# JosephCatrambone/aruco3

Measured on AMD Instinct MI355X. Metric: frames/sec at 1920x1080 ARUCO dict, higher is better.
Workload: dtype u8

## Files before the change

aruco3_amd/csrc/a3_api.hip:

```cpp
#include <algorithm>
#include <atomic>
#include <cmath>
#include <chrono>
#include <cstddef>
#include <cstdio>
#include <cstring>
#include <mutex>
#include <string>
#include <vector>

#include "a3_common.h"
#include "a3_internal.h"

namespace a3 {
hipError_t launch_grey_threshold(hipStream_t, const uint8_t*, int, size_t, size_t, int, int, uint32_t, uint32_t, uint8_t*, uint64_t*, uint16_t*);
bool threshold_writes_grey_plane(uint32_t radius, const uint8_t* pixels, size_t row_stride, size_t frame_stride, int W);
hipError_t launch_dart_count(hipStream_t, const uint64_t*, int, int, uint32_t, uint32_t, unsigned long long*, uint32_t*, uint64_t, uint32_t*, uint32_t*, void*, size_t);
size_t tile_darts_bytes(uint32_t W, uint32_t H, uint32_t n_frames);
size_t tile_off_offset(uint32_t W, uint32_t H, uint32_t n_frames);
size_t tile_mask_offset_bytes(uint32_t W, uint32_t H, uint32_t n_frames);
hipError_t launch_dart_build(hipStream_t, const uint64_t*, int, int, uint32_t, uint32_t, const uint32_t*, const uint32_t*, uint32_t*, const uint32_t*,
                             uint64_t*, uint32_t*, uint32_t, const uint32_t*, int, const unsigned long long*);
hipError_t launch_zero(hipStream_t, void*, size_t);
size_t entry_state_bytes();
bool finalize_inline(bool frame_entries, bool trust_natural);
size_t fin_state_bytes();
size_t entry_slots(uint32_t);
size_t leader_list_bytes(uint32_t);
hipError_t launch_rank_cycles(hipStream_t, uint32_t, int, const uint64_t*, const uint32_t*,
                              uint32_t*, unsigned int*, void*, void*, void*, uint32_t*, unsigned int*, int, DeviceCounters*, const uint32_t*, int,
                              const uint32_t*, uint32_t*, uint32_t, int, uint32_t, unsigned int*, int);
hipError_t launch_resolve(hipStream_t, const void*, uint32_t, int, const uint64_t*, const uint32_t*, const unsigned int*, uint64_t*, uint64_t*,
                          DeviceCounters*, int, const uint32_t*);
hipError_t launch_select_scatter(hipStream_t, const void*, uint32_t, const uint32_t*, const unsigned int*, const uint32_t*, const uint64_t*,
                                 const uint32_t*, uint32_t, uint32_t,
                                 uint32_t, double, double, ContourRec*, uint32_t*, uint32_t, uint64_t, DeviceCounters*,
                                 const uint64_t*, uint32_t*, const uint32_t*, int, uint32_t*, int, const void*);
hipError_t launch_debug_clockwise(hipStream_t, const int32_t*, uint32_t, int32_t*);
hipError_t launch_unpack_bits(hipStream_t, const uint64_t*, int, int, uint8_t*);
hipError_t launch_contour_quads(hipStream_t, const ContourRec*, const DeviceCounters*, uint32_t, const uint32_t*, double, uint32_t, uint32_t,
                                uint32_t, CandRec*, uint32_t*, unsigned int*, int, uint32_t);
size_t decode_out_bytes();
hipError_t launch_frame_candidates(hipStream_t, const CandRec*, const uint32_t*, uint32_t, uint32_t, float, uint16_t*, uint16_t*, uint32_t*,
                                   uint32_t*, unsigned int*, uint32_t, void*, float*);
uint32_t frame_cand_lds_slots();
size_t proj_rec_bytes();
size_t weight_table_bytes();
hipError_t launch_weight_table(hipStream_t, uint32_t, uint32_t, uint32_t, float*);
hipError_t launch_decode(hipStream_t, PixelSrc, int, int, uint32_t, const uint16_t*, const uint32_t*, const unsigned int*, uint32_t,
                         uint32_t, uint32_t, uint32_t, const uint64_t*, uint32_t, uint32_t, int, void*, const float*, void*, uint8_t*, uint32_t, uint32_t*, int, int, int);
hipError_t launch_compact_markers(hipStream_t, const void*, const uint16_t*, const uint32_t*, uint32_t, uint32_t, uint32_t, a3_marker*,
                                  uint32_t, uint32_t*, unsigned int*, unsigned int*, const uint32_t*, unsigned int*);
hipError_t launch_pack_detections(hipStream_t, const a3_marker*, const a3_pose*, const uint32_t*, uint32_t, uint32_t, uint32_t, void*, unsigned int*);
hipError_t launch_debug_rotate_bits(hipStream_t, const uint8_t*, uint32_t, uint32_t, uint8_t*);
hipError_t launch_gather_patches(hipStream_t, const void*, uint32_t, const uint8_t*, uint32_t, uint32_t, uint8_t*, unsigned int*);
hipError_t launch_pose(hipStream_t, const uint32_t*, uint32_t, const float*, uint32_t, const unsigned int*, int, float, float, float, float,
                       float, float, float, a3_pose*);
hipError_t launch_find_nearest(hipStream_t, const uint64_t*, uint32_t, const uint64_t*, uint32_t, uint32_t*, uint8_t*);
size_t refine_params_bytes();
void refine_params(void*, const a3_refine_config&, uint32_t);
hipError_t launch_refine_corners(hipStream_t, PixelSrc, uint32_t, uint32_t, const a3_marker*, const unsigned int*, const float*, const float*, uint32_t,
                                 const void*, float*);
size_t board_slot_bytes();
void board_slot_from(const float*, void*);
hipError_t launch_board_pose(hipStream_t, const a3_marker*, const uint32_t*, const float*, const float*, const unsigned int*, const uint32_t*,
                             uint32_t, uint32_t, const uint16_t*, uint32_t, const void*, const a3_intrinsics*, uint32_t, uint32_t, a3_board_pose*);
hipError_t launch_undistort_corners(hipStream_t, const a3_marker*, const float*, const unsigned int*, uint32_t, const a3_intrinsics&,
                                    const a3_distortion&, float*, float*);
hipError_t launch_charuco_corners(hipStream_t, PixelSrc, uint32_t, uint32_t, const a3_marker*, const uint32_t*, const float*, const float*,
                                  const unsigned int*, const uint32_t*, uint32_t, uint32_t, const uint16_t*, uint32_t, const void*, const float*,
                                  const uint32_t*, uint32_t, uint32_t, uint32_t, const void*, const a3_intrinsics*, const a3_distortion*,
                                  a3_charuco_corner*, uint32_t*, a3_charuco_corner*, float*);
hipError_t launch_charuco_pose(hipStream_t, const a3_marker*, const float*, const unsigned int*, const uint32_t*, uint32_t, uint32_t, const uint16_t*,
                               uint32_t, const void*, const float*, uint32_t, const uint32_t*, const a3_charuco_corner*, const float*,
                               const a3_intrinsics*, uint32_t, uint32_t, a3_charuco_pose*);
hipError_t launch_calc_tau(hipStream_t, const uint64_t*, uint32_t, unsigned int*);
size_t rig_obs_bytes();
size_t rig_frame_bytes();
size_t rig_table_bytes();
hipError_t launch_rig(hipStream_t, const a3_rig*, uint32_t, const a3_rig_camera*, const a3_rig_observation*, const float*, const float*, uint32_t*,
                      double*, double*, a3_rig_result*, a3_rig_camera_result*, a3_rig_frame*, a3_rig_observation_result*);
size_t calib_view_bytes();
hipError_t launch_calibrate(hipStream_t, const a3_calib_camera*, uint32_t, const uint32_t*, const float*, const float*, double*, a3_calib_result*,
                            a3_calib_view*);
hipError_t launch_synth_render(hipStream_t, const a3_synth_frame*, uint32_t, const a3_synth_marker*, uint32_t, uint32_t, int, float, float, int,
                               uint8_t*, size_t, size_t);
hipError_t launch_spin(hipStream_t, int, int, int, uint32_t*);
hipError_t launch_selftest(hipStream_t, const double*, const double*, uint32_t, double*, double*, float*, float*);
}

using namespace a3;

namespace {

thread_local std::string g_create_error;

constexpr uint32_t kMaxCandDefault = 1024, kMaxCandLimit = A3_MAX_CANDIDATES_PER_FRAME;
static_assert(kMaxCandLimit == 65536, "a3_marker.candidate_index is a uint16_t");
constexpr uint32_t kMaxContoursDefault = 1u << 20;
constexpr uint64_t kMaxDartsDefault = 48ull << 20;
constexpr uint64_t kMaxPointsDefault = 64ull << 20;
constexpr uint64_t kHardMaxDarts = (1ull << 30) - (1ull << 16);
constexpr uint64_t kHardMaxPoints = 3ull << 30;
constexpr int kResolveItersMax = 16;
constexpr uint32_t kPatchCapMin = 32768, kPatchCapMax = 1u << 20;

struct DevBuf {
    void* p = nullptr;
    size_t cap = 0;
    hipError_t ensure(size_t bytes) {
        if (bytes <= cap) return hipSuccess;
        if (p) { hipError_t e = hipFree(p); p = nullptr; cap = 0; if (e != hipSuccess) return e; }
        hipError_t e = hipMalloc(&p, bytes);
        if (e == hipSuccess) cap = bytes;
        return e;
    }
    void release() { if (p) (void)hipFree(p); p = nullptr; cap = 0; }
    template <typename T> T* as() const { return reinterpret_cast<T*>(p); }
};

struct Chunk { uint32_t first, count; uint64_t darts; uint32_t max_frame_darts; };
struct Batch {
    const uint8_t* pixels = nullptr; int fmt = 0;
    uint32_t W = 0, H = 0, n = 0;
    size_t row_stride = 0, frame_stride = 0, out_cap = 0;
    bool want_pose = false, pose_has_intr = false;
    float pose_size_mm = 0.0f;
    a3_intrinsics pose_intr{};
    size_t pose_bytes = 0;
    a3_refine_config refine{};
    size_t refine_bytes = 0;
    bool board = false;
// ... 202 lines not shown
bool g_hold_rests = true;
std::atomic<int> g_jump_rounds_cap{0};
enum { kStreamCopy = 0, kStreamDecode = 1 };

hipError_t create_stream(hipStream_t* st) { return hipStreamCreateWithPriority(st, hipStreamNonBlocking, 0); }

hipError_t device_stream(int device, int kind, hipStream_t* out) {
    std::lock_guard<std::mutex> lk(g_streams_mu);
    DeviceStreams& ds = g_dev_streams[device & 63];
    hipStream_t& st = kind == kStreamDecode ? ds.decode : ds.copy;
    if (!st) {
        const hipError_t e = create_stream(&st);
        if (e != hipSuccess) { st = nullptr; return e; }
    }
    *out = st;
    return hipSuccess;
}

int need_stream(a3_ctx* ctx);

std::mutex g_defer_mu;
std::vector<a3_ctx*> g_deferred;
std::atomic<int> g_overlap_force{-1};
std::vector<a3_ctx*> g_contexts;
int batch_mode_of(const a3_ctx* ctx) {
    const int f = g_overlap_force.load(std::memory_order_relaxed);
    if (f >= 0) return f;
    if (!ctx->stream || ctx->stream == ctx->own_stream) return 0;
    std::lock_guard<std::mutex> lk(g_streams_mu);
    for (const a3_ctx* o : g_contexts)
        if (o != ctx && o->device == ctx->device && o->stream == ctx->stream) return 2;
    return 0;
}
int release_mode() {
    const int f = g_overlap_force.load(std::memory_order_relaxed);
    return f >= 0 ? f : 2;
}

const void* refine_params_for(a3_ctx* ctx, const a3_refine_config& cfg) {
    if (ctx->refine_prm.empty() || memcmp(&ctx->refine_prm_cfg, &cfg, sizeof cfg) != 0) {
        ctx->refine_prm.assign((refine_params_bytes() + 3) / 4, 0.0f);
        refine_params(ctx->refine_prm.data(), cfg, ctx->mark_size);
        ctx->refine_prm_cfg = cfg;
    }
    return ctx->refine_prm.data();
}

size_t charuco_slot_bytes(const Batch& b) { return ((size_t)b.n * b.charuco_nc * sizeof(a3_charuco_corner) + 255) & ~(size_t)255; }
size_t charuco_stage_off(const Batch& b) {
    return b.head_bytes + (size_t)b.guess * (sizeof(a3_marker) + b.pose_bytes + b.refine_bytes + b.undist_bytes) +
           (b.board ? (size_t)b.n * sizeof(a3_board_pose) : 0);
}
size_t charuco_stage_bytes(const Batch& b) {
    return b.charuco ? 16 + (size_t)b.charuco_guess * sizeof(a3_charuco_corner) + (b.want_pose ? (size_t)b.n * sizeof(a3_charuco_pose) : 0) : 0;
}
const void* charuco_params_for(a3_ctx* ctx, const a3_charuco_config& cfg) {
    if (ctx->charuco_prm.empty() || memcmp(&ctx->charuco_prm_cfg, &cfg, sizeof cfg) != 0) {
        ctx->charuco_prm.assign((refine_params_bytes() + 3) / 4, 0.0f);
        const a3_refine_config rc{A3_REFINE_SUBPIX, cfg.win_half, cfg.relative_win, cfg.max_iterations, cfg.min_shift};
        refine_params(ctx->charuco_prm.data(), rc, 0);
        ctx->charuco_prm_cfg = cfg;
    }
    return ctx->charuco_prm.data();
}

int enqueue_back(a3_ctx* ctx, hipStream_t st, const Batch& b) {
    const uint32_t S = ctx->cfg.homography_sample_size;
    const float min_corner_separation = (float)std::min(b.W, b.H) * ctx->cfg.min_corner_separation_factor;
    unsigned int* d_work_count = ctx->scratch_u32 + 0;
    unsigned int* d_marker_total = ctx->scratch_u32 + 1;
    unsigned int* d_err = ctx->scratch_u32 + 4;
    if (ctx->inject_armed) {
        ctx->inject_armed = false;
        const uint32_t cnt = (uint32_t)ctx->inject.size();
        if (cnt) A3_HIP(hipMemcpyAsync(ctx->cands.p, ctx->inject.data(), cnt * sizeof(CandRec), hipMemcpyHostToDevice, st));
        ctx->inject_count = cnt;
        A3_HIP(hipMemcpyAsync(ctx->cand_count, &ctx->inject_count, 4, hipMemcpyHostToDevice, st));
    }
    A3_HIP(launch_frame_candidates(st, ctx->cands.as<CandRec>(), ctx->cand_count, b.n, b.max_cand, min_corner_separation,
                                   ctx->pre_xy.as<uint16_t>(), ctx->fin_xy.as<uint16_t>(), ctx->fin_count.as<uint32_t>(),
                                   ctx->work.as<uint32_t>(), d_work_count, S, ctx->proj.p, ctx->cand_big.as<float>()));
    const int few = b.n <= 64u ? 1 : 0;
    A3_HIP(launch_decode(st, b.src, (int)b.W, (int)b.H, 0, ctx->fin_xy.as<uint16_t>(), ctx->work.as<uint32_t>(), d_work_count,
                         b.max_cand, S, ctx->mark_size, S, ctx->dict.as<uint64_t>(), ctx->n_codes, ctx->tau, ctx->cfg.filter_high_bit_errors,
                         ctx->proj.p, ctx->wtab.as<float>(), ctx->outs.p, b.taps ? ctx->patches.as<uint8_t>() : nullptr, b.patch_cap, ctx->per_frame,
                         (int)std::min<uint32_t>(4096u, b.n * 128u) , 0,
                         few));
    A3_HIP(launch_compact_markers(st, ctx->outs.p, ctx->fin_xy.as<uint16_t>(), ctx->fin_count.as<uint32_t>(), b.n, 0, b.max_cand,
                                  ctx->markers_ptr, b.marker_cap, ctx->per_frame, d_marker_total, d_err, ctx->cand_count, ctx->scratch_u32 + 2));
    if (b.refine_bytes)
        A3_HIP(launch_refine_corners(st, b.src, b.W, b.H, ctx->markers_ptr, d_marker_total, nullptr, nullptr, b.marker_cap,
                                     refine_params_for(ctx, b.refine), ctx->refined_buf.as<float>()));
    if (b.undist_bytes)
        A3_HIP(launch_undistort_corners(st, ctx->markers_ptr, b.refine_bytes ? ctx->refined_buf.as<float>() : nullptr, d_marker_total, b.marker_cap,
                                        b.pose_intr, b.dist, ctx->undist_buf.as<float>(), ctx->undist_buf.as<float>() + (size_t)b.marker_cap * 8));
    const float* fcorners = b.undist_bytes ? ctx->undist_buf.as<float>() : b.refine_bytes ? ctx->refined_buf.as<float>() : nullptr;
    const uint32_t* charuco_counts = b.charuco ? reinterpret_cast<const uint32_t*>(ctx->charuco_tmp.as<uint8_t>() + charuco_slot_bytes(b)) : nullptr;
    float* charuco_und = b.charuco && b.want_pose && b.undist_bytes ? ctx->charuco_und.as<float>() : nullptr;
    if (b.charuco)
        A3_HIP(launch_charuco_corners(st, b.src, b.W, b.H, ctx->markers_ptr, nullptr, nullptr, b.refine_bytes ? ctx->refined_buf.as<float>() : nullptr,
                                      d_marker_total, ctx->per_frame, b.marker_cap, b.n, ctx->board_slot_of.as<uint16_t>(), ctx->n_codes,
                                      ctx->board_slot_rec.p, ctx->charuco_tab.as<float>(), ctx->charuco_tab.as<uint32_t>() + 2 * (size_t)b.charuco_nc,
                                      b.charuco_nc, b.charuco_cfg.min_markers, b.charuco_cfg.refine, charuco_params_for(ctx, b.charuco_cfg),
                                      &b.pose_intr, &b.dist, ctx->charuco_tmp.as<a3_charuco_corner>(), const_cast<uint32_t*>(charuco_counts),
                                      ctx->charuco_buf.as<a3_charuco_corner>(), charuco_und));
    if (b.want_pose) {
        const a3_intrinsics& in = b.pose_intr;
        if (fcorners)
            A3_HIP(launch_pose(st, nullptr, 8u, fcorners, b.marker_cap, d_marker_total, b.pose_has_intr ? 4 : 3, b.pose_size_mm,
                               (float)b.W, (float)b.H, in.focal_x, in.focal_y, in.principal_x, in.principal_y, ctx->pose_buf.as<a3_pose>()));
        else
            A3_HIP(launch_pose(st, reinterpret_cast<const uint32_t*>(reinterpret_cast<const uint8_t*>(ctx->markers_ptr) + offsetof(a3_marker, corners)),
                               (uint32_t)(sizeof(a3_marker) / 4), nullptr, b.marker_cap, d_marker_total, b.pose_has_intr ? 1 : 0, b.pose_size_mm,
                               (float)b.W, (float)b.H, in.focal_x, in.focal_y, in.principal_x, in.principal_y, ctx->pose_buf.as<a3_pose>()));
        if (b.board)
            A3_HIP(launch_board_pose(st, ctx->markers_ptr, nullptr, nullptr, fcorners, d_marker_total,
                                     ctx->per_frame, b.marker_cap, b.n, ctx->board_slot_of.as<uint16_t>(), ctx->n_codes, ctx->board_slot_rec.p,
                                     b.pose_has_intr ? &in : nullptr, b.W, b.H, ctx->board_buf.as<a3_board_pose>()));
        if (b.charuco)
            A3_HIP(launch_charuco_pose(st, ctx->markers_ptr, fcorners, d_marker_total, ctx->per_frame, b.marker_cap, b.n,
                                       ctx->board_slot_of.as<uint16_t>(), ctx->n_codes, ctx->board_slot_rec.p, ctx->charuco_tab.as<float>(),
                                       b.charuco_nc, charuco_counts, ctx->charuco_buf.as<a3_charuco_corner>(), charuco_und,
                                       b.pose_has_intr ? &in : nullptr, b.W, b.H, ctx->charuco_pose_buf.as<a3_charuco_pose>()));
    }
    if (b.prof >= 2) A3_HIP(hipEventRecord(ctx->ev[3], st));
    uint8_t* hp = (uint8_t*)ctx->pinned;
    a3_pose* h_poses = reinterpret_cast<a3_pose*>(hp + b.head_bytes + (size_t)b.guess * sizeof(a3_marker));
    A3_HIP(hipMemcpyAsync(hp, ctx->scratch_u32, b.head_bytes + (size_t)b.guess * sizeof(a3_marker), hipMemcpyDeviceToHost, st));
    if (b.pose_bytes) A3_HIP(hipMemcpyAsync(h_poses, ctx->pose_buf.p, (size_t)b.guess * b.pose_bytes, hipMemcpyDeviceToHost, st));
    if (b.refine_bytes)
        A3_HIP(hipMemcpyAsync(reinterpret_cast<uint8_t*>(h_poses) + (size_t)b.guess * b.pose_bytes, ctx->refined_buf.p, (size_t)b.guess * b.refine_bytes,
                              hipMemcpyDeviceToHost, st));
    if (b.board)
        A3_HIP(hipMemcpyAsync(reinterpret_cast<uint8_t*>(h_poses) + (size_t)b.guess * (b.pose_bytes + b.refine_bytes), ctx->board_buf.p,
                              (size_t)b.n * sizeof(a3_board_pose), hipMemcpyDeviceToHost, st));
    if (b.undist_bytes) {
        uint8_t* hu = reinterpret_cast<uint8_t*>(h_poses) + (size_t)b.guess * (b.pose_bytes + b.refine_bytes) + (b.board ? (size_t)b.n * sizeof(a3_board_pose) : 0);
        A3_HIP(hipMemcpyAsync(hu, ctx->undist_buf.p, (size_t)b.guess * 32, hipMemcpyDeviceToHost, st));
        A3_HIP(hipMemcpyAsync(hu + (size_t)b.guess * 32, ctx->undist_buf.as<float>() + (size_t)b.marker_cap * 8, (size_t)b.guess * 16,
                              hipMemcpyDeviceToHost, st));
    }
    if (b.charuco) {
        uint8_t* hc = hp + charuco_stage_off(b);
        A3_HIP(hipMemcpyAsync(hc, charuco_counts + b.n, 4, hipMemcpyDeviceToHost, st));
        A3_HIP(hipMemcpyAsync(hc + 16, ctx->charuco_buf.p, (size_t)b.charuco_guess * sizeof(a3_charuco_corner), hipMemcpyDeviceToHost, st));
        if (b.want_pose)
            A3_HIP(hipMemcpyAsync(hc + 16 + (size_t)b.charuco_guess * sizeof(a3_charuco_corner), ctx->charuco_pose_buf.p,
                                  (size_t)b.n * sizeof(a3_charuco_pose), hipMemcpyDeviceToHost, st));
    }
    if (b.taps) {
        A3_HIP(hipMemcpyAsync(ctx->pinned_counts, ctx->cand_count, (size_t)b.n * 4, hipMemcpyDeviceToHost, st));
        A3_HIP(hipMemcpyAsync((uint8_t*)ctx->pinned_counts + (size_t)b.n * 4, ctx->fin_count.p, (size_t)b.n * 4, hipMemcpyDeviceToHost, st));
    }
    A3_HIP(hipEventRecord(ctx->ev[4], st));
    return A3_OK;
}

int flush_deferred_impl(a3_ctx* ctx, hipEvent_t after);
int flush_deferred_locked(a3_ctx* ctx, hipEvent_t after) {
    const int rc = flush_deferred_impl(ctx, after);
    if (rc) ctx->back_rc = rc;
    return rc;
}
int flush_deferred_impl(a3_ctx* ctx, hipEvent_t after) {
    if (!ctx->back_deferred) return A3_OK;
    ctx->back_deferred = false;
    for (size_t i = 0; i < g_deferred.size(); i++)
// ... 193 lines not shown
        ctx->per_frame = reinterpret_cast<uint32_t*>(z + head_off + 256 + ctr_bytes);
        ctx->markers_ptr = reinterpret_cast<a3_marker*>(z + head_off + head_bytes);
        zero_p = z; zero_bytes = (head_off + head_bytes + 15) & ~(size_t)15;
        return launch ? launch_zero(st, zero_p, zero_bytes) : hipSuccess;
    };
    std::vector<Chunk> chunks;
    std::vector<uint64_t> fd;
    if (device_plan) {
        if (int rc = ensure_chain_buffers(ctx, st, b, cap_d)) return rc;
        chunks.push_back(Chunk{0, n, cap_d, (uint32_t)std::min<uint64_t>(cap_d, 0xFFFFFFFFu)});
        A3_HIP(layout_zero_block(1, n, false));
        ctx->frame_darts_ptr = ctx->frame_darts_dev.as<unsigned long long>();
    } else {
        A3_HIP(ctx->tile_darts.ensure(tile_darts_bytes(W, H, n)));
        ctx->frame_darts_ptr = ctx->frame_darts.as<unsigned long long>();
        A3_HIP(hipMemsetAsync(ctx->frame_darts.p, 0, (size_t)n * 8, st));
    }
    A3_HIP(launch_dart_count(st, ctx->bin.as<uint64_t>(), (int)W, (int)H, 0, n, ctx->frame_darts_ptr, ctx->tile_darts.as<uint32_t>(), cap_d,
                             device_plan ? ctx->frame_base.as<uint32_t>() : nullptr, device_plan ? ctx->scratch_u32 + 8 : nullptr,
                             device_plan ? zero_p : nullptr, device_plan ? zero_bytes : 0));
    const uint32_t* n_live = device_plan ? ctx->scratch_u32 + 8 : nullptr;
    uint32_t max_chunk_frames = n;
    if (!device_plan) {
        if (int rc = ensure_pinned(ctx, std::max<size_t>((size_t)n * 8, 1 << 16))) return rc;
        A3_HIP(hipMemcpyAsync(ctx->pinned, ctx->frame_darts.p, (size_t)n * 8, hipMemcpyDeviceToHost, st));
        A3_HIP(wait_stream(st));
        fd.assign((uint64_t*)ctx->pinned, (uint64_t*)ctx->pinned + n);
        uint64_t biggest = 0;
        for (uint64_t v : fd) { biggest = std::max(biggest, v); ctx->stats.darts += v; }
        if (biggest > kHardMaxDarts) return fail(ctx, A3_ERR_LIMIT, "a frame needs more contour-graph nodes than 32-bit indices allow");
        if (biggest > ctx->max_darts) ctx->max_darts = biggest;
        Chunk c{0, 0, 0, 0};
        for (uint32_t f = 0; f < n; f++) {
            if (c.count && (c.darts + fd[f] > ctx->max_darts || c.count >= kMaxChunkFrames)) { chunks.push_back(c); c = Chunk{f, 0, 0, 0}; }
            c.count++; c.darts += fd[f]; c.max_frame_darts = (uint32_t)std::max<uint64_t>(c.max_frame_darts, fd[f]);
        }
        if (c.count) chunks.push_back(c);
        max_chunk_frames = 0; uint64_t max_chunk_darts = 0;
        for (auto& c : chunks) { max_chunk_frames = std::max(max_chunk_frames, c.count); max_chunk_darts = std::max(max_chunk_darts, c.darts); }
        if (int rc = ensure_dart_pool(ctx, pool_darts_of(ctx, max_chunk_darts, chunks.size()))) return rc;
        A3_HIP(ctx->pix_base.ensure((size_t)max_chunk_frames * npx * 4));
        A3_HIP(ctx->frame_base.ensure((size_t)(max_chunk_frames + 1) * 4 * chunks.size()));
        A3_HIP(layout_zero_block(chunks.size(), max_chunk_frames, true));
        A3_HIP(ctx->contours.ensure((size_t)ctx->max_contours * sizeof(ContourRec)));
        A3_HIP(ctx->cyc_start_off.ensure((size_t)ctx->max_contours * 4));
        A3_HIP(ctx->points.ensure(ctx->max_points * 4));
        std::vector<uint32_t> bases;
        for (auto& c : chunks) {
            uint32_t acc = 0;
            for (uint32_t i = 0; i < max_chunk_frames + 1; i++) {
                bases.push_back(acc);
                if (i < c.count) acc += (uint32_t)fd[c.first + i];
            }
        }
        if (int rc = ensure_pinned(ctx, (size_t)n * 8 + bases.size() * 4 + (1 << 16))) return rc;
        uint32_t* h_bases = reinterpret_cast<uint32_t*>((uint8_t*)ctx->pinned + (size_t)n * 8);
        memcpy(h_bases, bases.data(), bases.size() * 4);
        A3_HIP(hipMemcpyAsync(ctx->frame_base.p, h_bases, bases.size() * 4, hipMemcpyHostToDevice, st));
    }
    ctx->stats.chunks = (uint32_t)chunks.size();

    unsigned int* d_err = ctx->scratch_u32 + 4;
    unsigned int* d_entry_count = ctx->scratch_u32 + 32;
    unsigned int* d_leader_count = ctx->scratch_u32 + 16;
    unsigned int* d_dead_count = ctx->scratch_u32 + 48;

    const uint64_t* d_bin = ctx->bin.as<uint64_t>();
    const double image_diag = std::sqrt((double)W * W + (double)H * H);
    const double eps_factor = ctx->cfg.contour_simplification_epsilon;
    const int resolve_iters = ctx->resolve_full_ttl > 0 ? ctx->resolve_iters_hint : 0;
    const int inline_resolve_W = ctx->resolve_full_ttl > 0 ? 0 : (int)W;
    const int keep_all = b.taps ? 1 : 0;
    int rounds_max = 0;
    for (size_t ci = 0; ci < chunks.size(); ci++) {
        const Chunk& c = chunks[ci];
        DeviceCounters* ctr = ctx->counters + ci;
        const uint32_t* fb = ctx->frame_base.as<uint32_t>() + ci * (max_chunk_frames + 1);
        const uint32_t nd = (uint32_t)c.darts;
        if (nd == 0) continue;
        if (ci > 0) {
            A3_HIP(hipMemsetAsync(d_leader_count, 0, 4 * 32, st));
            A3_HIP(hipMemsetAsync(ctx->frame_cursor, 0, (size_t)c.count * 4, st));
        }
        const uint32_t* tile_off = ctx->tile_darts.as<uint32_t>() + tile_off_offset(W, H, n);
        A3_HIP(launch_dart_build(st, d_bin, (int)W, (int)H, c.first, c.count, fb, tile_off, ctx->pix_base.as<uint32_t>(),
                                 ctx->tile_darts.as<uint32_t>(), ctx->d_xy.as<uint64_t>(), ctx->d_succ.as<uint32_t>(), nd, n_live, 0,
                                 reinterpret_cast<const unsigned long long*>(ctx->tile_darts.as<uint8_t>() + tile_mask_offset_bytes(W, H, n))));
        int rounds = 1;
        while ((1ull << rounds) < (uint64_t)c.max_frame_darts && rounds < 31) rounds++;
        rounds += 1;
        rounds = std::min(rounds, ctx->jump_rounds_hint);
        if (const int cap = g_jump_rounds_cap.load(std::memory_order_relaxed); cap > 0 && ctx->jump_rounds_hint < 32) rounds = std::min(rounds, cap);
        rounds_max = std::max(rounds_max, rounds);
        uint32_t* const frame_entries = ctx->entry_global_ttl > 0 ? nullptr : ctx->frame_cursor;
        const bool dense_graph = (uint64_t)nd * 10u >= (uint64_t)c.count * npx;
        unsigned int* const dead_ctr = (keep_all || !dense_graph) ? nullptr : d_dead_count;
        A3_HIP(launch_rank_cycles(st, nd, (int)W, ctx->d_xy.as<uint64_t>(), ctx->d_succ.as<uint32_t>(),
                                  ctx->entry_list.as<uint32_t>(), d_entry_count, ctx->es_a.p, ctx->es_b.p,
                                  ctx->fin.p, ctx->leader_list.as<uint32_t>(), d_leader_count, rounds, ctr, n_live, 0, fb,
                                  frame_entries, c.count, 1, min_edge_length, dead_ctr, inline_resolve_W > 0 ? 1 : 0));
        if (rel_mode == 2) { if (int rc = release_waiting()) return rc; }
        ctx->dbg_nd = nd; ctx->dbg_frames = c.count; ctx->dbg_chunks = (uint32_t)chunks.size();
        A3_HIP(launch_rank_cycles(st, nd, (int)W, ctx->d_xy.as<uint64_t>(), ctx->d_succ.as<uint32_t>(),
                                  ctx->entry_list.as<uint32_t>(), d_entry_count, ctx->es_a.p, ctx->es_b.p,
                                  ctx->fin.p , ctx->leader_list.as<uint32_t>(), d_leader_count, rounds, ctr,
                                  n_live, 0, fb, frame_entries, c.count, 2, min_edge_length, dead_ctr, inline_resolve_W > 0 ? 1 : 0));
        const void* fin = ctx->fin.p;
        A3_HIP(launch_resolve(st, fin, nd, (int)W, ctx->d_xy.as<uint64_t>(), ctx->leader_list.as<uint32_t>(), d_leader_count,
                              ctx->t_cur.as<uint64_t>(), ctx->t_next.as<uint64_t>(), ctr, resolve_iters, n_live));
        A3_HIP(launch_select_scatter(st, fin, nd, ctx->leader_list.as<uint32_t>(), d_leader_count, ctx->d_succ.as<uint32_t>(), ctx->t_cur.as<uint64_t>(), fb,
                                     c.count, c.first, min_edge_length, eps_factor, image_diag,
                                     ctx->contours.as<ContourRec>(), ctx->cyc_start_off.as<uint32_t>(), ctx->max_contours, ctx->max_points, ctr,
                                     ctx->d_xy.as<uint64_t>(), ctx->points.as<uint32_t>(), n_live, inline_resolve_W, ctx->leader_keep.as<uint32_t>(),
                                     keep_all, finalize_inline(frame_entries != nullptr, inline_resolve_W > 0) ? ctx->es_a.p : nullptr));
        A3_HIP(launch_contour_quads(st, ctx->contours.as<ContourRec>(), ctr, ctx->max_contours, ctx->points.as<uint32_t>(),
                                    eps_factor, min_edge_length, c.first, kMaxCand,
                                    ctx->cands.as<CandRec>() + (size_t)c.first * kMaxCand, ctx->cand_count + c.first, d_err,
                                    W <= 16384u && H <= 16384u ? 1 : 0, nd));
    }
    if (rel_mode != 0) { if (int rc = release_waiting()) return rc; }
    if (b.prof >= 2) A3_HIP(hipEventRecord(ctx->ev[2], st));

    b.src = b.need_grey ? PixelSrc{ctx->grey.as<uint8_t>(), W, (unsigned long long)npx, kFmtGreyPlane}
                        : PixelSrc{b.pixels, b.row_stride, b.frame_stride, b.fmt};
    ctx->dbg_src = b.src;
    b.head_bytes = head_bytes;
    if (int rc = ensure_back_buffers(ctx, b, head_bytes)) return rc;
    b.device_plan = device_plan; b.n_chunks = chunks.size(); b.chunk0_darts = chunks.empty() ? 0 : chunks[0].darts;
    b.ctr_bytes = ctr_bytes; b.rounds_max = rounds_max;
    ctx->counts_valid = false;
    if (ctx->allow_defer && !defer_locked && b.profiling < 2 && ctx->batch_mode != 0) {
        A3_HIP(hipEventRecord(ctx->ev_contours, st));
        std::lock_guard<std::mutex> lk(g_defer_mu);
        ctx->back_deferred = true;
        ctx->back_rc = 0;
        ctx->stepping = A3_STEP_DECODE_DEFERRED;
        g_deferred.push_back(ctx);
    } else if (int rc = enqueue_back(ctx, st, b)) return rc;
    b.active = true;
    return A3_OK;
}

int enqueue_batch(a3_ctx* ctx) {
    ctx->stepping = A3_STEP_WHOLE;
    if (int rc = enqueue_front(ctx, ctx->batch, false)) return rc;
    return enqueue_chain(ctx, ctx->batch, false);
}

int finish_batch(a3_ctx* ctx, a3_marker* out, a3_pose* poses, size_t out_cap, uint32_t* per_frame_count, size_t* out_n) {
    Batch& b = ctx->batch;
    if (!b.active) return fail(ctx, A3_ERR_INVALID, "no batch was submitted");
    {
        std::lock_guard<std::mutex> lk(g_defer_mu);
        (void)flush_held_locked(ctx, nullptr);
        if (const int rc = ctx->held_rc) { ctx->held_rc = 0; b.active = false; return rc; }
    }
    b.active = false;
    hipStream_t st = ctx->stream;
    const size_t ctr_bytes = b.ctr_bytes, head_bytes = b.head_bytes, pose_bytes = b.pose_bytes, n_chunks = b.n_chunks, refine_bytes = b.refine_bytes;
    const size_t undist_bytes = b.undist_bytes, board_bytes = b.board ? (size_t)b.n * sizeof(a3_board_pose) : 0;
    const uint32_t guess = b.guess, n = b.n;
    uint8_t* hp = (uint8_t*)ctx->pinned;
    a3_marker* h_markers = reinterpret_cast<a3_marker*>(hp + head_bytes);
    a3_pose* h_poses = reinterpret_cast<a3_pose*>(hp + head_bytes + (size_t)guess * sizeof(a3_marker));
    const float* h_refined = reinterpret_cast<const float*>(hp + head_bytes + (size_t)guess * (sizeof(a3_marker) + pose_bytes));
    const float* h_undist = reinterpret_cast<const float*>(hp + head_bytes + (size_t)guess * (sizeof(a3_marker) + pose_bytes + refine_bytes) + board_bytes);
    const float* h_undist_res = h_undist + (size_t)guess * 8;
    {
        std::lock_guard<std::mutex> lk(g_defer_mu);
        if (int rc = flush_deferred_locked(ctx, nullptr)) return rc;
// ... 543 lines not shown
        ctx->stepping = A3_STEP_BURST_LAST; ctx->released_others = released;
        return erc;
    }
    ctx->allow_defer = true;
    const int erc = enqueue_batch(ctx);
    ctx->allow_defer = false;
    return erc;
}

static int collect_common(a3_ctx* ctx, a3_marker* out, a3_pose* poses, size_t out_cap, uint32_t* per_frame_count, size_t* out_n) {
    *out_n = 0;
    if (ctx->pending_trivial) {
        ctx->pending_trivial = false;
        finish_trivial(ctx, per_frame_count);
        return A3_OK;
    }
    A3_HIP(hipSetDevice(ctx->device));
    if (int rcs_ = need_stream(ctx)) return rcs_;
    int rc = finish_batch(ctx, out, poses, out_cap, per_frame_count, out_n);
    const uint32_t stepping = ctx->stepping;
    if (rc == 1) { ctx->reruns++; ctx->batch.out_cap = out_cap; rc = run_batch_with_retries(ctx, out, poses, out_cap, per_frame_count, out_n); }
    ctx->stepping = stepping;
    return rc;
}

int a3_detect_batch_submit(a3_ctx* ctx, const void* pixels, int memory, int fmt, uint32_t width, uint32_t height, size_t row_stride,
                           size_t frame_stride, uint32_t n_frames, size_t out_cap) {
    if (!ctx) return A3_ERR_INVALID;
    return submit_common(ctx, pixels, memory, fmt, width, height, row_stride, frame_stride, n_frames, out_cap, false, 0.0f, nullptr);
}

int a3_detect_batch_collect(a3_ctx* ctx, a3_marker* out, size_t out_cap, uint32_t* per_frame_count, size_t* out_n) {
    if (!ctx) return A3_ERR_INVALID;
    if (!out_n || (!out && out_cap)) return fail(ctx, A3_ERR_INVALID, "a3_detect_batch_collect: null output");
    return collect_common(ctx, out, nullptr, out_cap, per_frame_count, out_n);
}

int a3_detect_batch_pose_submit(a3_ctx* ctx, const void* pixels, int memory, int fmt, uint32_t width, uint32_t height, size_t row_stride,
                                size_t frame_stride, uint32_t n_frames, float marker_size_mm, const a3_intrinsics* intr, size_t out_cap) {
    if (!ctx) return A3_ERR_INVALID;
    return submit_common(ctx, pixels, memory, fmt, width, height, row_stride, frame_stride, n_frames, out_cap, true, marker_size_mm, intr);
}

int a3_detect_batch_pose_collect(a3_ctx* ctx, a3_marker* out, a3_pose* poses, size_t out_cap, uint32_t* per_frame_count, size_t* out_n) {
    if (!ctx) return A3_ERR_INVALID;
    if (!out_n || (!out && out_cap) || (!poses && out_cap)) return fail(ctx, A3_ERR_INVALID, "a3_detect_batch_pose_collect: null output");
    if (!ctx->pending_trivial && ctx->batch.active && !ctx->batch.want_pose)
        return fail(ctx, A3_ERR_INVALID, "a3_detect_batch_pose_collect: the submitted batch was not an a3_detect_batch_pose_submit call");
    return collect_common(ctx, out, poses, out_cap, per_frame_count, out_n);
}

int a3_detect_batch_pose(a3_ctx* ctx, const void* pixels, int memory, int fmt, uint32_t width, uint32_t height, size_t row_stride,
                         size_t frame_stride, uint32_t n_frames, float marker_size_mm, const a3_intrinsics* intr, a3_marker* out,
                         a3_pose* poses, size_t out_cap, uint32_t* per_frame_count, size_t* out_n) {
    if (!ctx || !poses) return A3_ERR_INVALID;
    return detect_common(ctx, pixels, memory, fmt, width, height, row_stride, frame_stride, n_frames, true, marker_size_mm, intr, out, poses,
                         out_cap, per_frame_count, out_n);
}

int a3_debug_kernel_time(a3_ctx* ctx, int kernel, int dbg, int reps, float* avg_ms) {
    if (!ctx || !avg_ms || reps <= 0) return A3_ERR_INVALID;
    if (ctx->dbg_chunks != 1 || ctx->dbg_nd == 0) return fail(ctx, A3_ERR_INVALID, "needs a preceding single-chunk batch");
    A3_HIP(hipSetDevice(ctx->device));
    if (int rcs_ = need_stream(ctx)) return rcs_;
    hipStream_t st = ctx->stream;
    struct EventPair {
        hipEvent_t e0 = nullptr, e1 = nullptr;
        ~EventPair() { if (e0) (void)hipEventDestroy(e0); if (e1) (void)hipEventDestroy(e1); }
    } evp;
    A3_HIP(hipEventCreate(&evp.e0)); A3_HIP(hipEventCreate(&evp.e1));
    const hipEvent_t e0 = evp.e0, e1 = evp.e1;
    double total = 0.0;
    unsigned int* d_entry_count = ctx->scratch_u32 + 32;
    unsigned int* d_leader_count = ctx->scratch_u32 + 16;
    for (int r = 0; r < reps; r++) {
        A3_HIP(hipMemsetAsync(d_leader_count, 0, 4 * 32, st));
        A3_HIP(hipEventRecord(e0, st));
        if (kernel == 0) {
            A3_HIP(hipMemsetAsync(ctx->frame_darts.p, 0, (size_t)ctx->frames * 8, st));
            A3_HIP(launch_dart_count(st, ctx->bin.as<uint64_t>(), (int)ctx->W, (int)ctx->H, 0, ctx->frames, ctx->frame_darts.as<unsigned long long>(),
                                     ctx->tile_darts.as<uint32_t>(), 0, nullptr, nullptr, nullptr, 0));
        } else if (kernel == 1) {
            A3_HIP(launch_dart_build(st, ctx->bin.as<uint64_t>(), (int)ctx->W, (int)ctx->H, 0, ctx->dbg_frames, ctx->frame_base.as<uint32_t>(),
                                     ctx->tile_darts.as<uint32_t>() + tile_off_offset(ctx->W, ctx->H, ctx->frames), ctx->pix_base.as<uint32_t>(),
                                     ctx->tile_darts.as<uint32_t>(), ctx->d_xy.as<uint64_t>(),
                                     ctx->d_succ.as<uint32_t>(), ctx->dbg_nd, nullptr, dbg ? dbg : 5,
                                     reinterpret_cast<const unsigned long long*>(ctx->tile_darts.as<uint8_t>() + tile_mask_offset_bytes(ctx->W, ctx->H, ctx->frames))));
        } else if (kernel == 2) {
            A3_HIP(launch_rank_cycles(st, ctx->dbg_nd, (int)ctx->W, ctx->d_xy.as<uint64_t>(), ctx->d_succ.as<uint32_t>(),
                                      ctx->entry_list.as<uint32_t>(),
                                      d_entry_count, ctx->es_a.p, ctx->es_b.p, ctx->fin.p,
                                      ctx->leader_list.as<uint32_t>(), d_leader_count, 0, ctx->counters, nullptr, dbg ? dbg : 11, ctx->frame_base.as<uint32_t>(), nullptr, ctx->dbg_frames, 0,
                                      0u, nullptr, 0));
        } else if (kernel == 3 || kernel == 4) {
            if (kernel == 4) {
                const size_t sweep = std::min<size_t>(ctx->pix_base.cap & ~(size_t)15, (size_t)512 << 20);
                if (sweep) A3_HIP(launch_zero(st, ctx->pix_base.p, sweep));
                A3_HIP(hipEventRecord(e0, st));
            }
            A3_HIP(launch_decode(st, ctx->dbg_src, (int)ctx->W, (int)ctx->H, 0, ctx->fin_xy.as<uint16_t>(), ctx->work.as<uint32_t>(), ctx->scratch_u32,
                                 ctx->max_cand, ctx->cfg.homography_sample_size, ctx->mark_size, ctx->cfg.homography_sample_size, ctx->dict.as<uint64_t>(),
                                 ctx->n_codes, ctx->tau, ctx->cfg.filter_high_bit_errors, ctx->proj.p, ctx->wtab.as<float>(), ctx->outs.p, nullptr, 0u, nullptr, 4096,
                                 dbg == 0 ? -1000 : dbg, ctx->frames <= 64u ? 1 : 0));
        } else return fail(ctx, A3_ERR_INVALID, "kernel: 0 dart_count, 1 dart_assign, 2 local_contract, 3 decode, 4 decode on cold frames");
        A3_HIP(hipEventRecord(e1, st));
        A3_HIP(hipStreamSynchronize(st));
        float ms = 0;
        A3_HIP(hipEventElapsedTime(&ms, e0, e1));
        total += ms;
    }
    *avg_ms = (float)(total / reps);
    return A3_OK;
}

int a3_debug_set_overlap(int mode) {
    if (mode < -1 || mode > 2) return A3_ERR_INVALID;
    std::lock_guard<std::mutex> lk(g_defer_mu);
    if (!g_held.empty() || !g_deferred.empty()) return A3_ERR_INVALID;
    g_overlap_force.store(mode, std::memory_order_relaxed);
    return A3_OK;
}

int a3_debug_spin(void* hip_stream, int workgroups, int threads, int usec) {
    if (workgroups < 1 || workgroups > 1024 || threads < 64 || threads > 512 || threads % 64 || usec < 1 || usec > 100000) return A3_ERR_INVALID;
    static uint32_t* sink = nullptr;
    static std::mutex mu;
    {
        std::lock_guard<std::mutex> lk(mu);
        if (!sink) {
            if (hipMalloc(&sink, 4096 * 4) != hipSuccess) return A3_ERR_HIP;
            if (hipMemset(sink, 0, 4096 * 4) != hipSuccess) return A3_ERR_HIP;
        }
    }
    return launch_spin(reinterpret_cast<hipStream_t>(hip_stream), workgroups, threads, usec, sink) == hipSuccess ? A3_OK : A3_ERR_HIP;
}

int a3_debug_build_flags(void) { return 0; }

int a3_debug_launch_threshold(a3_ctx* ctx, const void* pixels_device, int fmt, uint32_t width, uint32_t height, uint32_t n_frames) {
    if (!ctx || !pixels_device || n_frames == 0) return A3_ERR_INVALID;
    A3_HIP(hipSetDevice(ctx->device));
    if (int rc = need_stream(ctx)) return rc;
    const size_t bpp = fmt == A3_FMT_RGB8 ? 3 : (fmt == A3_FMT_L8 ? 1 : 4);
    if (threshold_writes_grey_plane(ctx->cfg.threshold_window, reinterpret_cast<const uint8_t*>(pixels_device), (size_t)width * bpp, (size_t)width * bpp * height, (int)width))
        return fail(ctx, A3_ERR_INVALID, "a3_debug_launch_threshold: this threshold_window / frame layout takes the separable path, which needs a grey plane");
    A3_HIP(ctx->bin.ensure((size_t)words_per_row(width) * 8 * height * n_frames));
    A3_HIP(launch_grey_threshold(ctx->stream, reinterpret_cast<const uint8_t*>(pixels_device), fmt, (size_t)width * bpp, (size_t)width * bpp * height,
                                 (int)width, (int)height, n_frames, ctx->cfg.threshold_window, nullptr, ctx->bin.as<uint64_t>(), nullptr));
    return A3_OK;
}

int a3_debug_set_hold(int on) {
    std::lock_guard<std::mutex> lk(g_defer_mu);
    if (!g_held.empty()) return A3_ERR_INVALID;
    g_hold_rests = on != 0;
    return A3_OK;
}

int a3_debug_set_jump_rounds(int rounds) {
    if (rounds < 0 || rounds > 32) return A3_ERR_INVALID;
    g_jump_rounds_cap.store(rounds, std::memory_order_relaxed);
    return A3_OK;
}

int a3_synth_render(int device, void* hip_stream, const a3_synth_frame* frames, uint32_t n_frames, const a3_synth_marker* markers,
                    uint32_t n_markers, uint32_t width, uint32_t height, int paper, float black, float white, int supersample,
                    void* out_rgb_device, size_t row_stride, size_t frame_stride) {
    if (!frames || !out_rgb_device || (n_markers && !markers) || supersample < 1 || supersample > 8) return A3_ERR_INVALID;
    if (n_frames == 0 || width == 0 || height == 0) return A3_OK;
    if (row_stride == 0) row_stride = (size_t)width * 3;
    if (frame_stride == 0) frame_stride = row_stride * height;
    if (row_stride < (size_t)width * 3 || frame_stride < row_stride * (height - 1) + (size_t)width * 3 || height > 65535 || n_frames > 65535)
        return A3_ERR_INVALID;
    for (uint32_t f = 0; f < n_frames; f++)
        if ((uint64_t)frames[f].first_marker + frames[f].n_markers > n_markers) return A3_ERR_INVALID;
    for (uint32_t m = 0; m < n_markers; m++)
        if (markers[m].n == 0 || markers[m].n > 11) return A3_ERR_INVALID;
    if (hipSetDevice(device) != hipSuccess) return A3_ERR_NO_DEVICE;
    hipStream_t st = reinterpret_cast<hipStream_t>(hip_stream);
    a3_synth_frame* d_frames = nullptr; a3_synth_marker* d_markers = nullptr;
    hipError_t e = hipMalloc(&d_frames, sizeof(a3_synth_frame) * n_frames);
    if (e == hipSuccess && n_markers) e = hipMalloc(&d_markers, sizeof(a3_synth_marker) * n_markers);
    if (e == hipSuccess) e = hipMemcpyAsync(d_frames, frames, sizeof(a3_synth_frame) * n_frames, hipMemcpyHostToDevice, st);
    if (e == hipSuccess && n_markers) e = hipMemcpyAsync(d_markers, markers, sizeof(a3_synth_marker) * n_markers, hipMemcpyHostToDevice, st);
// ... 853 lines not shown
```

aruco3_amd/csrc/k_contours.hip:

```cpp
#include <algorithm>

#include "a3_common.h"


namespace a3 {

constexpr int kFinB = 8;
constexpr int kScatB = 1;

struct Nb8 { uint64_t c; uint64_t n[8]; };

__device__ __forceinline__ uint64_t ldw(const uint64_t* __restrict__ img, int wpr, int H, int j, int y) {
    return (y >= 0 && y < H && j >= 0 && j < wpr) ? img[(size_t)y * wpr + j] : 0ull;
}

__device__ __forceinline__ void pdart_words(const Nb8& nb, uint64_t p[8]) {
#pragma unroll
    for (int k = 0; k < 8; k++) {
        uint64_t m = nb.c & nb.n[k] & ~nb.n[(k + 7) & 7];
        if ((k & 1) == 0) m &= ~nb.n[(k + 6) & 7];
        p[k] = m;
    }
}

__device__ __forceinline__ uint32_t block_excl_scan_256(uint32_t v, uint32_t* s_wave, uint32_t* total) {
    const int lane = threadIdx.x & 63, wave = threadIdx.x >> 6;
    uint32_t inc = v;
#define A3_DPP_ADD(CTRL, ROWMASK) inc += (uint32_t)__builtin_amdgcn_update_dpp(0, (int)inc, CTRL, ROWMASK, 0xF, false);
    A3_DPP_ADD(0x111, 0xF)
    A3_DPP_ADD(0x112, 0xF)
    A3_DPP_ADD(0x114, 0xF)
    A3_DPP_ADD(0x118, 0xF)
    A3_DPP_ADD(0x142, 0xA)
    A3_DPP_ADD(0x143, 0xC)
#undef A3_DPP_ADD
    if (lane == 63) s_wave[wave] = inc;
    __syncthreads();
    uint32_t base = 0, tot = 0;
#pragma unroll
    for (int w = 0; w < 4; w++) {
        const uint32_t t = s_wave[w];
        if (w < wave) base += t;
        tot += t;
    }
    *total = tot;
    return base + inc - v;
}

constexpr int kTileWords = 4, kTileRows = 64;
__host__ __device__ inline uint32_t dart_tiles_x(uint32_t W) { return (words_per_row(W) + kTileWords - 1) / kTileWords; }
__host__ __device__ inline uint32_t dart_tiles(uint32_t W, uint32_t H) { return dart_tiles_x(W) * ((H + kTileRows - 1) / kTileRows); }

__device__ __forceinline__ void tile_stage(const uint64_t* __restrict__ img, int W, int H, uint32_t tile, uint64_t (*s_t)[kTileWords + 2]) {
    const int wpr = (int)words_per_row((uint32_t)W);
    const int tx = tile % dart_tiles_x((uint32_t)W), ty = tile / dart_tiles_x((uint32_t)W);
    const int j0 = tx * kTileWords - 1, y0 = ty * kTileRows - 1;
    constexpr int kStage = (kTileRows + 2) * (kTileWords + 2);
    static_assert(kStage <= 512, "two words per lane");
    uint64_t v[2];
#pragma unroll
    for (int k = 0; k < 2; k++) {
        const int i = min((int)threadIdx.x + 256 * k, kStage - 1);
        const int r = i / (kTileWords + 2), c = i - r * (kTileWords + 2);
        const int jj = j0 + c, yy = y0 + r;
        const uint64_t w = img[(size_t)min(max(yy, 0), H - 1) * wpr + min(max(jj, 0), wpr - 1)];
        v[k] = w & (0ull - (uint64_t)(yy >= 0 && yy < H && jj >= 0 && jj < wpr));
    }
#pragma unroll
    for (int k = 0; k < 2; k++) {
        const int i = (int)threadIdx.x + 256 * k;
        if (i < kStage) (&s_t[0][0])[i] = v[k];
    }
}
__device__ __forceinline__ Nb8 tile_nb8(const uint64_t (*s_t)[kTileWords + 2], int rl, int jl) {
    Nb8 r;
    const uint64_t al = s_t[rl][jl], a = s_t[rl][jl + 1], ar = s_t[rl][jl + 2];
    const uint64_t cl = s_t[rl + 1][jl], c = s_t[rl + 1][jl + 1], cr = s_t[rl + 1][jl + 2];
    const uint64_t bl = s_t[rl + 2][jl], b = s_t[rl + 2][jl + 1], br = s_t[rl + 2][jl + 2];
    r.c = c;
    r.n[0] = (c << 1) | (cl >> 63);
    r.n[1] = (a << 1) | (al >> 63);
    r.n[2] = a;
    r.n[3] = (a >> 1) | (ar << 63);
    r.n[4] = (c >> 1) | (cr << 63);
    r.n[5] = (b >> 1) | (br << 63);
    r.n[6] = b;
    r.n[7] = (b << 1) | (bl >> 63);
    return r;
}

constexpr int kCountLanes = 60;
constexpr int kCountHalves = 4;
template <int G>
__global__ __launch_bounds__(64) void k_dart_count(const uint64_t* __restrict__ bits, int W, int H, uint32_t first_frame,
                                                   unsigned long long* __restrict__ frame_darts, uint32_t* __restrict__ tile_darts,
                                                   uint32_t* __restrict__ tile_darts_h1, unsigned long long* __restrict__ tile_mask) {
    static_assert(kCountLanes % kTileWords == 0, "a wave counts whole tiles");
    static_assert((kTileRows / kCountHalves) * kTileWords == 64, "one 64-bit mask per tile and part");
    constexpr int kGroups = 64 / G, kOwners = G == 64 ? kCountLanes : 30, kTilesPerGroup = (kOwners + kTileWords - 1) / kTileWords;
    __shared__ uint32_t s_tile[kGroups][kTilesPerGroup];
    __shared__ unsigned long long s_mask[kGroups][kTilesPerGroup];
    constexpr uint32_t kQ = 128;
    __shared__ uint64_t q_c[kQ], q_up[kQ], q_dn[kQ];
    __shared__ uint32_t q_meta[kQ];
    const int wpr = (int)words_per_row((uint32_t)W);
    const uint32_t f = blockIdx.y;
    const uint32_t tiles_x = dart_tiles_x((uint32_t)W), tiles_y = ((uint32_t)H + kTileRows - 1) / kTileRows;
    const int chunks_x = G == 64 ? (wpr + kCountLanes - 1) / kCountLanes : 1;
    const int lane = threadIdx.x, gl = lane & (G - 1), grp = lane / G;
    const int cx = blockIdx.x % chunks_x, ty = (blockIdx.x / chunks_x) * kGroups + grp;
    const int j = cx * kOwners + gl - 1;
    const bool owner = gl >= 1 && gl <= kOwners && j < wpr && ty < (int)tiles_y;
    const uint64_t* img = bits + (size_t)(first_frame + f) * wpr * H;
    if (lane < kGroups * kTilesPerGroup) { (&s_tile[0][0])[lane] = 0; (&s_mask[0][0])[lane] = 0ull; }
    constexpr int kRows = kTileRows / kCountHalves;
    const int y0 = ty * kTileRows + (int)blockIdx.z * kRows;
    const int jc = min(max(j, 0), wpr - 1);
    auto word = [&](int y) -> uint64_t {
        const uint64_t v = img[(size_t)min(max(y, 0), H - 1) * wpr + jc];
        return v & (0ull - (uint64_t)(y >= 0 && y < H && j >= 0 && j < wpr));
    };
    auto edge_bits = [](uint64_t c, uint32_t* lr) {
        const uint32_t l = (uint32_t)__builtin_amdgcn_update_dpp(0, (int)(uint32_t)(c >> 32), 0x138 , 0xF, 0xF, true) >> 31;
        const uint32_t r = (uint32_t)__builtin_amdgcn_update_dpp(0, (int)(uint32_t)c, 0x130 , 0xF, 0xF, true) & 1u;
        *lr = l | (r << 1);
    };
    struct Row3 { uint64_t c; uint32_t lr; };
    constexpr int kAhead = 16;
    static_assert(kRows % kAhead == 0, "whole batches of rows");
    Row3 up, cur;
    uint64_t nxt[kAhead], ahead[kAhead];
    up.c = word(y0 - 1);
    cur.c = word(y0);
#pragma unroll
    for (int u = 0; u < kAhead; u++) nxt[u] = word(y0 + u + 1);
    edge_bits(up.c, &up.lr);
    edge_bits(cur.c, &cur.lr);
    uint32_t qhead = 0, qtail = 0;
    const uint32_t lane_row0 = (uint32_t)lane << 8;
    auto work = [&](uint32_t slot) {
        const uint64_t c = q_c[slot], uc = q_up[slot], dc = q_dn[slot];
        const uint32_t m = q_meta[slot];
        Nb8 nb;
        nb.c = c;
        nb.n[0] = (c << 1) | (m & 1u);                  nb.n[4] = (c >> 1) | ((uint64_t)((m >> 1) & 1u) << 63);
        nb.n[1] = (uc << 1) | ((m >> 2) & 1u);          nb.n[3] = (uc >> 1) | ((uint64_t)((m >> 3) & 1u) << 63);
        nb.n[2] = uc;                                   nb.n[6] = dc;
        nb.n[7] = (dc << 1) | ((m >> 4) & 1u);          nb.n[5] = (dc >> 1) | ((uint64_t)((m >> 5) & 1u) << 63);
        uint64_t p[8];
        pdart_words(nb, p);
// ... 21 lines not shown
            const uint64_t c = cur.c;
            const bool white = (c & up.c & dn.c) == ~0ull && (cur.lr & up.lr & dn.lr) == 3u;
            const bool hot = owner && c != 0ull && !white;
            const unsigned long long bal = __ballot(hot);
            if (bal) {
                if (hot) {
                    const uint32_t below = __builtin_amdgcn_mbcnt_hi((uint32_t)(bal >> 32), __builtin_amdgcn_mbcnt_lo((uint32_t)bal, 0u));
                    const uint32_t slot = (qtail + below) & (kQ - 1);
                    q_c[slot] = c; q_up[slot] = up.c; q_dn[slot] = dn.c;
                    q_meta[slot] = cur.lr | (up.lr << 2) | (dn.lr << 4) | lane_row0 | ((uint32_t)(r0 + u) << 16);
                }
                qtail += (uint32_t)__popcll(bal);
                if (qtail - qhead >= 64u) {
                    wave_sync();
                    work((qhead + (uint32_t)lane) & (kQ - 1));
                    qhead += 64u;
                    wave_sync();
                }
            }
            up = cur; cur = dn;
        }
#pragma unroll
        for (int u = 0; u < kAhead; u++) nxt[u] = ahead[u];
    }
    wave_sync();
    if ((uint32_t)lane < qtail - qhead) work((qhead + (uint32_t)lane) & (kQ - 1));
    __builtin_amdgcn_s_waitcnt(0);
    __builtin_amdgcn_wave_barrier();
    uint32_t total = 0;
    if (gl < kTilesPerGroup && ty < (int)tiles_y) {
        const uint32_t tx = (uint32_t)(cx * kTilesPerGroup + gl);
        if (tx < tiles_x) {
            total = s_tile[grp][gl];
            (blockIdx.z ? tile_darts_h1 + (size_t)(blockIdx.z - 1) * gridDim.y * (tiles_x * tiles_y) : tile_darts)[(size_t)(first_frame + f) * (tiles_x * tiles_y) + ty * tiles_x + tx] = total;
        }
    }
    if (gl >= 1 && gl <= kOwners && ((gl - 1) & (kTileWords - 1)) == 0 && ty < (int)tiles_y) {
        const uint32_t tx = (uint32_t)(cx * kTilesPerGroup + (gl - 1) / kTileWords);
        if (tx < tiles_x) tile_mask[((size_t)(first_frame + f) * (tiles_x * tiles_y) + ty * tiles_x + tx) * kCountHalves + blockIdx.z] = s_mask[grp][(gl - 1) / kTileWords];
    }
#define A3_DPP_ADD(CTRL, ROWMASK) total += (uint32_t)__builtin_amdgcn_update_dpp(0, (int)total, CTRL, ROWMASK, 0xF, false);
    A3_DPP_ADD(0x111, 0xF) A3_DPP_ADD(0x112, 0xF) A3_DPP_ADD(0x114, 0xF) A3_DPP_ADD(0x118, 0xF) A3_DPP_ADD(0x142, 0xA) A3_DPP_ADD(0x143, 0xC)
#undef A3_DPP_ADD
    if (lane == 63 && total) atomicAdd(&frame_darts[f], (unsigned long long)total);
}

__device__ void plan_frames(unsigned long long* __restrict__ frame_darts, uint32_t n_frames, unsigned long long cap,
                            uint32_t* __restrict__ frame_base, uint32_t* __restrict__ plan) {
    __shared__ unsigned long long s_pw[4];
    __shared__ unsigned long long s_run;
    __shared__ unsigned int s_max;
    const int lane = threadIdx.x & 63, wave = threadIdx.x >> 6;
    if (threadIdx.x == 0) { s_run = 0; s_max = 0; }
    __syncthreads();
    for (uint32_t base = 0; base < n_frames; base += 256) {
        const uint32_t i = base + threadIdx.x;
        const unsigned long long v = i < n_frames ? frame_darts[i] : 0ull;
        if (i < n_frames) frame_darts[i] = 0ull;
        unsigned long long inc = v;
#pragma unroll
        for (int o = 1; o < 64; o <<= 1) { const unsigned long long t = __shfl_up(inc, o); if (lane >= o) inc += t; }
        if (lane == 63) s_pw[wave] = inc;
        atomicMax(&s_max, (unsigned int)min(v, 0xFFFFFFFFull));
        __syncthreads();
        unsigned long long before = s_run, tot = 0;
        for (int w = 0; w < 4; w++) { const unsigned long long t = s_pw[w]; if (w < wave) before += t; tot += t; }
        if (i < n_frames) frame_base[i] = (uint32_t)min(before + inc - v, 0xFFFFFFFFull);
        __syncthreads();
        if (threadIdx.x == 0) s_run += tot;
        __syncthreads();
    }
    if (threadIdx.x == 0) {
        const unsigned long long total = s_run;
        const bool fits = total <= cap;
        frame_base[n_frames] = fits ? (uint32_t)total : 0u;
        plan[0] = fits ? (uint32_t)total : 0u;
        plan[1] = fits ? 0u : 1u;
        plan[2] = s_max;
        plan[3] = (uint32_t)min(total, 0xFFFFFFFFull);
    }
}

__global__ __launch_bounds__(256) void k_tile_scan(uint32_t* __restrict__ tile_darts, const uint32_t* __restrict__ tile_darts_h1, uint32_t tiles, uint32_t first_frame,
                                                   uint32_t* __restrict__ tile_off, uint32_t n_frames,
                                                   unsigned long long* __restrict__ frame_darts, unsigned long long cap,
                                                   uint32_t* __restrict__ frame_base, uint32_t* __restrict__ plan,
                                                   uint4* __restrict__ zero_p, uint32_t zero_n16) {
    if (blockIdx.x == n_frames) {
        for (uint32_t i = threadIdx.x; i < zero_n16; i += 256) zero_p[i] = make_uint4(0u, 0u, 0u, 0u);
        __syncthreads();
        plan_frames(frame_darts, n_frames, cap, frame_base, plan);
        return;
    }
    __shared__ uint32_t s_wave[4];
    __shared__ uint32_t s_run;
    const size_t base = (size_t)(first_frame + blockIdx.x) * tiles;
    if (threadIdx.x == 0) s_run = 0;
    __syncthreads();
    for (uint32_t t0 = 0; t0 < tiles; t0 += 256) {
        const uint32_t t = t0 + threadIdx.x;
        uint32_t v = 0;
        if (t < tiles) {
            v = tile_darts[base + t];
#pragma unroll
            for (int z = 1; z < kCountHalves; z++) v += tile_darts_h1[(size_t)(z - 1) * n_frames * tiles + base + t];
        }
        if (t < tiles) tile_darts[base + t] = v;
        uint32_t total;
        const uint32_t excl = block_excl_scan_256(v, s_wave, &total);
        if (t < tiles) tile_off[base + t] = s_run + excl;
        __syncthreads();
        if (threadIdx.x == 0) s_run += total;
        __syncthreads();
    }
}

__device__ __forceinline__ uint32_t row3(uint64_t l, uint64_t c, uint64_t r, int i) {
    const uint64_t v = i == 0 ? ((c << 1) | (l >> 63)) : (c >> (i - 1));
    return ((uint32_t)v & 7u) | (i == 63 ? ((uint32_t)r & 1u) << 2 : 0u);
}
__device__ __forceinline__ uint32_t tile_F(const uint64_t (*s_t)[kTileWords + 2], int rl, int jl, int i) {
    const uint32_t* base = reinterpret_cast<const uint32_t*>(&s_t[0][0]);
    const int p1 = (jl + 1) * 64 + i - 1, d = p1 >> 5, sh = p1 & 31;
    constexpr int kRowDwords = 2 * (kTileWords + 2);
    uint32_t rows[3];
#pragma unroll
    for (int k = 0; k < 3; k++) {
        const uint32_t* r = base + (rl + k) * kRowDwords + d;
        rows[k] = __builtin_amdgcn_alignbit(r[1], r[0], (uint32_t)sh) & 7u;
    }
    const uint32_t top = rows[0], mid = rows[1], bot = rows[2];
    return (mid & 1u) | ((top & 7u) << 1) | ((mid & 4u) << 2) | ((bot & 4u) << 3) | ((bot & 2u) << 5) | ((bot & 1u) << 7);
}
__device__ __forceinline__ int select_bit(uint64_t m, uint32_t r) {
    uint32_t w = (uint32_t)m, c = (uint32_t)__popc(w), pos = 0;
    if (r >= c) { w = (uint32_t)(m >> 32); r -= c; pos = 32; }
    c = (uint32_t)__popc(w & 0xFFFFu); if (r >= c) { w >>= 16; r -= c; pos += 16; }
    c = (uint32_t)__popc(w & 0xFFu);   if (r >= c) { w >>= 8;  r -= c; pos += 8; }
    c = (uint32_t)__popc(w & 0xFu);    if (r >= c) { w >>= 4;  r -= c; pos += 4; }
    c = (uint32_t)__popc(w & 3u);      if (r >= c) { w >>= 2;  r -= c; pos += 2; }
    return (int)(pos + (r >= (w & 1u) ? 1u : 0u));
}
struct PixLut { uint16_t v[256]; };
constexpr PixLut make_pix_lut() {
    PixLut t{};
    for (uint32_t F = 0; F < 256; F++) {
        const uint32_t rot1 = ((F << 1) | (F >> 7)) & 0xFFu, rot2 = ((F << 2) | (F >> 6)) & 0xFFu;
        const uint32_t P = F & ~rot1 & (0xAAu | ~rot2) & 0xFFu;
        uint32_t kW = 15, kE = 15;
        if (!(F & 1u)) { kW = 0; for (uint32_t b = 0; b < 7; b++) if ((F >> 1) & (1u << b)) { kW = b + 1; break; } }
        if (!(F & 16u)) {
            const uint32_t rr = ((F >> 5) | (F << 3)) & 0xFFu;
            uint32_t first = 0;
            for (uint32_t b = 0; b < 8; b++) if (rr & (1u << b)) { first = b + 1; break; }
            kE = (5 + first - 1) & 7;
        }
        t.v[F] = (uint16_t)(P | (kW << 8) | (kE << 12));
    }
    return t;
}
__device__ __constant__ const PixLut kPixLut = make_pix_lut();

__device__ __forceinline__ int dir_dx(int k) { return (int)((0x1A90u >> (2 * k)) & 3u) - 1; }
__device__ __forceinline__ int dir_dy(int k) { return (int)((0xA901u >> (2 * k)) & 3u) - 1; }

__global__ __launch_bounds__(256) void k_dart_assign(const uint64_t* __restrict__ bits, int W, int H, uint32_t first_frame,
                                                     const uint32_t* __restrict__ frame_base, const uint32_t* __restrict__ tile_off,
                                                     uint32_t* __restrict__ pix_base, const uint32_t* __restrict__ tile_darts,
                                                     uint64_t* __restrict__ d_rec, uint32_t* __restrict__ d_succ,
                                                     const uint32_t* __restrict__ n_live, int dbg,
                                                     const unsigned long long* __restrict__ tile_mask, uint32_t tiles, uint32_t n_frames) {
    __shared__ uint32_t s_wave[4];
    __shared__ uint64_t s_t[kTileRows + 2][kTileWords + 2];
    __shared__ uint64_t s_nodes[256];
    __shared__ uint64_t s_c0[256], s_c1[256], s_c2[256];
    __shared__ uint32_t s_dbase[256];
    __shared__ uint32_t s_mark[512];
    __shared__ uint16_t s_nbk[256];
    __shared__ uint8_t s_wofrank[256], s_rank[256], s_fr[256];
    __shared__ uint32_t s_multi;
    __shared__ uint16_t s_lut[256];
    const int wpr = (int)words_per_row((uint32_t)W);
    const uint32_t n_wg = tiles * n_frames, chunk = (n_wg + 7u) >> 3, g = (blockIdx.x & 7u) * chunk + (blockIdx.x >> 3);
    if (g >= n_wg) return;
    const uint32_t f = g / tiles, tile = g - f * tiles;
    if (tile_darts[(size_t)(first_frame + f) * tiles + tile] == 0u) return;
    if (n_live && *n_live == 0u) return;
    const uint32_t dart0 = frame_base[f] + tile_off[(size_t)(first_frame + f) * tiles + tile];
    if (dbg == 1) return;
    __shared__ uint32_t s_cnt[256];
    const unsigned long long* tm = tile_mask + ((size_t)(first_frame + f) * tiles + tile) * kCountHalves;
    static_assert(kCountHalves == 4 && kTileWords == 4 && kTileRows == 64, "four 64-bit word masks per tile, four word columns of 64 rows");
    unsigned long long cm[4];
#pragma unroll
    for (int c = 0; c < 4; c++)
        cm[c] = ((tm[0] >> (16 * c)) & 0xFFFFull) | (((tm[1] >> (16 * c)) & 0xFFFFull) << 16) | (((tm[2] >> (16 * c)) & 0xFFFFull) << 32) | (((tm[3] >> (16 * c)) & 0xFFFFull) << 48);
    const unsigned long long m0 = cm[0], m1 = cm[1], m2 = cm[2], m3 = cm[3];
    tile_stage(bits + (size_t)(first_frame + f) * wpr * H, W, H, tile, s_t);
    s_cnt[threadIdx.x] = 0;
    s_mark[threadIdx.x] = 0; s_mark[256 + threadIdx.x] = 0;
    s_lut[threadIdx.x] = kPixLut.v[threadIdx.x];
    if (threadIdx.x == 0) s_multi = 0;
    __syncthreads();
    const uint32_t a0 = (uint32_t)__popcll(m0), a1 = a0 + (uint32_t)__popcll(m1), a2 = a1 + (uint32_t)__popcll(m2), n_act = a2 + (uint32_t)__popcll(m3);
    for (uint32_t k = threadIdx.x; k < n_act; k += 256) {
        const uint32_t part = (k >= a0) + (k >= a1) + (k >= a2);
        const unsigned long long mm = part == 0 ? m0 : (part == 1 ? m1 : (part == 2 ? m2 : m3));
        const uint32_t w = part * 64u + (uint32_t)select_bit(mm, k - (part == 0 ? 0u : (part == 1 ? a0 : (part == 2 ? a1 : a2))));
        const Nb8 nb = tile_nb8(s_t, (int)(w & 63u), (int)(w >> 6));
        uint64_t p[8];
        pdart_words(nb, p);
        uint64_t nodes = 0;
        uint32_t nd = 0;
#pragma unroll
        for (int q = 0; q < 8; q++) { nd += __popcll(p[q]); nodes |= p[q]; }
        const uint64_t s1 = p[0] ^ p[1] ^ p[2], k1 = (p[0] & p[1]) | (p[2] & (p[0] ^ p[1]));
        const uint64_t s2 = p[3] ^ p[4] ^ p[5], k2 = (p[3] & p[4]) | (p[5] & (p[3] ^ p[4]));
        const uint64_t s3 = p[6] ^ p[7], k3 = p[6] & p[7];
        const uint64_t k4 = (s1 & s2) | (s3 & (s1 ^ s2));
        const uint64_t t = k1 ^ k2 ^ k3, q1 = (k1 & k2) | (k3 & (k1 ^ k2));
        s_nodes[w] = nodes;
        const uint64_t c1 = t ^ k4, c2 = q1 | (t & k4);
        s_c0[w] = s1 ^ s2 ^ s3; s_c1[w] = c1; s_c2[w] = c2;
        if ((c1 | c2) != 0ull) s_multi = 1u;
        s_cnt[w] = nd | ((uint32_t)__popcll(nodes) << 17);
        s_wofrank[k] = (uint8_t)w; s_rank[w] = (uint8_t)k;
    }
    __syncthreads();
    uint32_t total_p;
    const uint32_t excl_p = block_excl_scan_256(s_cnt[threadIdx.x], s_wave, &total_p);
    const uint32_t excl_d = excl_p & 0x1FFFFu, excl_n = excl_p >> 17, total_n = total_p >> 17;
    s_dbase[threadIdx.x] = excl_d;
    {
        const uint32_t cw = s_cnt[threadIdx.x] >> 17;
        if (cw) {
            const uint32_t k = s_rank[threadIdx.x];
            s_nbk[k] = (uint16_t)excl_n;
            if (excl_n) atomicOr(&s_mark[(excl_n - 1u) >> 5], 1u << ((excl_n - 1u) & 31u));
            const uint32_t seg = (excl_n + 63u) >> 6;
            if ((seg << 6) < excl_n + cw) s_fr[seg] = (uint8_t)k;
        }
    }
    if (dbg == 2) return;
    __syncthreads();
    if (dbg == 3) return;
    const int tx = tile % dart_tiles_x((uint32_t)W), ty = tile / dart_tiles_x((uint32_t)W);
    uint32_t* pbf = pix_base + (size_t)f * W * H;
    const bool single = __builtin_amdgcn_readfirstlane((int)s_multi) == 0;
    for (uint32_t n = threadIdx.x; n < total_n; n += 256) {
        const uint32_t seg = n >> 6;
        const uint32_t marks_below = __builtin_amdgcn_mbcnt_hi(s_mark[2u * seg + 1u], __builtin_amdgcn_mbcnt_lo(s_mark[2u * seg], 0u));
        const uint32_t kr = (uint32_t)s_fr[seg] + marks_below;
        const uint32_t w = s_wofrank[kr], r = n - (uint32_t)s_nbk[kr];
        const uint64_t m = s_nodes[w];
        const int i = select_bit(m, r);
        const int jl = w >> 6, rl = w & 63;
        const int wj = tx * kTileWords + jl, wy = ty * kTileRows + rl;
        const uint32_t F = tile_F(s_t, rl, jl, i);
        const uint32_t lut = s_lut[F];
        uint32_t P = lut & 0xFFu;
        const uint64_t below = (1ull << i) - 1ull;
        const uint32_t off = single ? (uint32_t)__popcll(m & below)
                                    : (uint32_t)__popcll(s_c0[w] & below) + 2u * (uint32_t)__popcll(s_c1[w] & below) + 4u * (uint32_t)__popcll(s_c2[w] & below);
        const int x = 64 * wj + i;
        uint32_t cur = dart0 + s_dbase[w] + off;
        if ((i == 0 || i == 63 || rl == 0 || rl == kTileRows - 1) && dbg != 4) pbf[(size_t)wy * W + x] = cur;
        const int kW = x > 0 ? (int)((lut >> 8) & 15u) : 15, kE = x + 1 < W ? (int)(lut >> 12) : 15;
        const uint32_t xy = (uint32_t)x | ((uint32_t)wy << 16);
        while (P) {
            const int k = __ffs(P) - 1;
            P &= P - 1;
            const uint32_t info = (uint32_t)k | (k == kW ? kInfoW : 0u) | (k == kE ? kInfoE : 0u);
            if (dbg != 4) d_rec[cur] = dart_rec(xy, F, info, f);
            const uint32_t rr = ((F >> k) | (F << (8 - k))) & 0xFFu;
            const int ko = (k + (31 - __clz(rr))) & 7, kin = (ko + 4) & 7;
            const int lx = jl * 64 + i + dir_dx(ko), ly = rl + dir_dy(ko);
            uint32_t succ;
            if (lx >= 0 && lx < kTileWords * 64 && ly >= 0 && ly < kTileRows) {
                const int j2 = lx >> 6, i2 = lx & 63, w2 = j2 * kTileRows + ly;
                const uint32_t P2 = (uint32_t)s_lut[tile_F(s_t, ly, j2, i2)] & 0xFFu;
                succ = cur;
                if ((P2 >> kin) & 1u) {
                    const uint64_t below2 = (1ull << i2) - 1ull;
                    const uint32_t off2 = single ? (uint32_t)__popcll(s_nodes[w2] & below2)
                                                 : (uint32_t)__popcll(s_c0[w2] & below2) + 2u * (uint32_t)__popcll(s_c1[w2] & below2) +
                                                   4u * (uint32_t)__popcll(s_c2[w2] & below2);
                    succ = dart0 + s_dbase[w2] + off2 + (uint32_t)__popc(P2 & ((1u << kin) - 1u));
                }
            } else {
                succ = kNone;
            }
            if (dbg != 4 || succ == 0x12345678u) d_succ[cur] = succ;
            cur++;
        }
    }
}

__device__ __forceinline__ uint32_t pixel_F(const uint64_t* __restrict__ img, int wpr, int H, int x, int y) {
    const int j = x >> 6, i = x & 63;
    uint32_t rows[3];
#pragma unroll
    for (int dy = -1; dy <= 1; dy++) {
        const uint64_t c = ldw(img, wpr, H, j, y + dy);
        const uint64_t l = i == 0 ? ldw(img, wpr, H, j - 1, y + dy) : 0ull;
        const uint64_t r = i == 63 ? ldw(img, wpr, H, j + 1, y + dy) : 0ull;
        rows[dy + 1] = row3(l, c, r, i);
    }
    const uint32_t top = rows[0], mid = rows[1], bot = rows[2];
    return (mid & 1u) | ((top & 7u) << 1) | ((mid & 4u) << 2) | ((bot & 4u) << 3) | ((bot & 2u) << 5) | ((bot & 1u) << 7);
}

__device__ __forceinline__ uint32_t cross_tile_succ(uint32_t d, uint64_t rec, int W, int H, int wpr, uint32_t first_frame,
                                                    const uint32_t* __restrict__ pix_base, const uint64_t* __restrict__ bits) {
    const uint32_t f = rec_frame(rec);
    const uint64_t* img = bits + (size_t)(first_frame + f) * wpr * H;
    const uint32_t* pb = pix_base + (size_t)f * W * H;
    const uint32_t xy = rec_xy(rec);
    const int x = xy & 0xFFFF, y = xy >> 16;
    const uint32_t F = rec_F(rec);
    const int k = rec_info(rec) & 7;
    const uint32_t r = ((F >> k) | (F << (8 - k))) & 0xFFu;
    const int ko = (k + (31 - __clz(r))) & 7;
    const int nx = x + dir_dx(ko), ny = y + dir_dy(ko);
    const uint32_t tP = pdart_mask(pixel_F(img, wpr, H, nx, ny));
    const int kin = (ko + 4) & 7;
    return ((tP >> kin) & 1u) ? pb[(size_t)ny * W + nx] + __popc(tP & ((1u << kin) - 1u)) : d;
}

__global__ __launch_bounds__(256) void k_dart_link(int W, int H, uint32_t first_frame, const uint32_t* __restrict__ pix_base,
                                                   const uint64_t* __restrict__ bits, const uint64_t* __restrict__ d_rec,
                                                   uint32_t* __restrict__ d_succ, uint32_t n_darts, const uint32_t* __restrict__ n_live) {
    if (n_live) n_darts = min(n_darts, *n_live);
    const int wpr = (int)words_per_row((uint32_t)W);
    constexpr int B = 8;
    const uint32_t stride = gridDim.x * blockDim.x;
    const uint32_t lane = threadIdx.x & 63u;
    for (uint32_t w0 = blockIdx.x * blockDim.x + (threadIdx.x & ~63u); w0 < n_darts; w0 += B * stride) {
        uint32_t sv[B];
#pragma unroll
        for (int u = 0; u < B; u++) sv[u] = d_succ[min(w0 + lane + (uint32_t)u * stride, n_darts - 1u)];
        uint64_t m[B];
        uint32_t total = 0;
#pragma unroll
        for (int u = 0; u < B; u++) {
            m[u] = __ballot(w0 + lane + (uint32_t)u * stride < n_darts && sv[u] == kNone);
            total += (uint32_t)__popcll(m[u]);
        }
        for (uint32_t j = lane; j < total; j += 64u) {
            uint32_t acc = 0, r = 0, su = 0;
            uint64_t mm = 0;
#pragma unroll
            for (int u = 0; u < B; u++) {
                const uint32_t c = (uint32_t)__popcll(m[u]);
                if (j >= acc && j < acc + c) { mm = m[u]; r = j - acc; su = (uint32_t)u; }
                acc += c;
            }
            const uint32_t d = w0 + (uint32_t)select_bit(mm, r) + su * stride;
            d_succ[d] = cross_tile_succ(d, d_rec[d], W, H, wpr, first_frame, pix_base, bits);
        }
    }
}

constexpr int kLT = 2048;
constexpr int kLTFrame = 1024;
constexpr uint32_t kEntryShards = 16;
constexpr uint32_t kLeaderShards = 16;
__host__ __device__ inline uint32_t leader_shard_cap(uint32_t n_darts) { return n_darts / kLeaderShards + n_darts / 64u + 262144u; }
__host__ __device__ inline uint32_t entry_shard_cap(uint32_t n_darts) {
    const uint32_t tiles = (n_darts + kLT - 1) / kLT;
    return ((tiles + kEntryShards - 1) / kEntryShards) * kLT;
}
struct EntrySpace {
    uint32_t cnt[kEntryShards], span, total;
    __device__ explicit EntrySpace(const unsigned int* __restrict__ entry_count) {
        uint32_t m = 0;
#pragma unroll
        for (uint32_t sh = 0; sh < kEntryShards; sh++) { cnt[sh] = entry_count[sh]; m = max(m, cnt[sh]); }
        span = max((m + 63u) & ~63u, 64u);
        total = span * kEntryShards;
    }
    __device__ uint32_t slot(uint32_t i0, uint32_t cap) const {
        const uint32_t sh = i0 / span, i = i0 - sh * span;
        uint32_t c = 0;
#pragma unroll
        for (uint32_t k = 0; k < kEntryShards; k++) c = (k == sh) ? cnt[k] : c;
        return i < c ? sh * cap + i : kNone;
    }
};
struct __attribute__((aligned(8))) FinState { uint32_t leader; uint32_t w; };
constexpr uint32_t kFinEvent = 0x80000000u, kFinDead = 0x40000000u, kFinHops = 0x3FFFFFFFu;
constexpr uint32_t kPend = 0x80000000u, kPendSlot = 0x3FFFFFFFu;
__device__ __forceinline__ bool is_pending(FinState s) { return (s.leader & kPend) != 0u; }
__device__ __forceinline__ FinState pend_pack(uint32_t slot, uint32_t dist, uint32_t off, uint32_t min_dart) {
    const uint32_t m = min_dart & 0x7FFu;
    return FinState{kPend | ((m >> 10) << 30) | (slot & kPendSlot), (dist - 1u) | (off << 11) | ((m & 0x3FFu) << 22)};
}
__device__ __forceinline__ uint32_t pend_slot(FinState s) { return s.leader & kPendSlot; }
__device__ __forceinline__ uint32_t pend_dist(FinState s) { return (s.w & 0x7FFu) + 1u; }
__device__ __forceinline__ uint32_t pend_off(FinState s) { return (s.w >> 11) & 0x7FFu; }
__device__ __forceinline__ uint32_t pend_min(FinState s, uint32_t d) { return (d & ~0x7FFu) | (((s.leader >> 30) & 1u) << 10) | (s.w >> 22); }
__device__ __forceinline__ uint32_t event_key(uint64_t rec, int W) {
    const uint32_t xy = rec_xy(rec), info = rec_info(rec);
    const uint32_t q = (xy >> 16) * (uint32_t)W + (xy & 0xFFFF);
    return (info & kInfoW) ? 2u * q : ((info & kInfoE) ? 2u * q + 1u : kNoKey);
}
__device__ __forceinline__ uint64_t dart_key(uint32_t d, uint64_t rec, int W) { return ((uint64_t)event_key(rec, W) << 32) | d; }

struct __attribute__((aligned(8))) EntryState { uint64_t key; uint32_t ptr; uint32_t off; uint32_t dist; uint32_t pad; };

__device__ __forceinline__ FinState resolve_pending(FinState s, uint32_t d, const EntryState& g) {
    const uint32_t leader = (uint32_t)g.key;
    const uint32_t hops = leader == pend_min(s, d) ? pend_off(s) : (pend_dist(s) + g.off) & kFinHops;
    return FinState{leader, hops | ((uint32_t)(g.key >> 32) != kNoKey ? kFinEvent : 0u)};
}
__device__ __forceinline__ EntryState entry_start(uint32_t e, FinState s, uint64_t min_rec, int W, uint32_t self) {
    EntryState r;
    const bool pend = is_pending(s);
    r.key = dart_key(pend ? pend_min(s, e) : s.leader, min_rec, W);
    r.off = pend ? pend_off(s) : (s.w & kFinHops);
    r.dist = pend ? pend_dist(s) : 0u;
    r.ptr = pend ? pend_slot(s) : self;
    r.pad = 0;
    return r;
}
__device__ __forceinline__ uint32_t entry_min_dart(uint32_t e, FinState s) { return is_pending(s) ? pend_min(s, e) : s.leader; }
__device__ __forceinline__ FinState fin_final(FinState s, uint32_t d, const EntryState* __restrict__ es) {
    return (es != nullptr && is_pending(s)) ? resolve_pending(s, d, es[pend_slot(s)]) : s;
}

__device__ __forceinline__ void lds_barrier() {
    __builtin_amdgcn_fence(__ATOMIC_RELEASE, "workgroup", "local");
    __builtin_amdgcn_s_barrier();
    __builtin_amdgcn_fence(__ATOMIC_ACQUIRE, "workgroup", "local");
}

__device__ __forceinline__ bool static_fire(uint64_t rec) {
    const uint32_t info = rec_info(rec), F = rec_F(rec);
    if (info & kInfoW) return __popc(pdart_mask(F)) == 1;
    if (info & kInfoE) return (rec_xy(rec) & 0xFFFFu) == 0u || (F & 1u) != 0u;
    return false;
}

template <int LT, bool DEAD >
__global__ __launch_bounds__(256, (LT >= 2048 || DEAD) ? 4 : 8) void k_local_contract(uint32_t n_darts, int W, const uint64_t* __restrict__ d_rec,
                                                        const uint32_t* __restrict__ d_succ,
                                                        FinState* __restrict__ fin,
                                                        uint32_t* __restrict__ entry_list,
                                                        unsigned int* __restrict__ entry_count, uint32_t ecap,
                                                        const uint32_t* __restrict__ frame_base, uint32_t* __restrict__ frame_entries,
                                                        const uint32_t* __restrict__ n_live, int dbg,
                                                        uint32_t min_edge_length, unsigned int* __restrict__ dead_count ,
                                                        int trust_natural ,
                                                        uint32_t* __restrict__ leader_list ,
                                                        unsigned int* __restrict__ leader_count , uint32_t leader_cap) {
    struct __attribute__((aligned(16))) Win { uint64_t key; uint32_t ptr; uint32_t offdist; };
    __shared__ Win s_win[LT];
    constexpr uint32_t kFrameWin = 64;
    __shared__ uint32_t s_fcnt[kFrameWin], s_fbase[kFrameWin];
    __shared__ uint32_t s_new_count, s_new_base, s_f0, s_dead_n;
    __shared__ __attribute__((aligned(4))) uint8_t s_dead[DEAD ? LT : 4];
    constexpr uint32_t kQCap = DEAD ? 1024 : 1;
    __shared__ uint32_t s_q[kQCap];
    __shared__ uint32_t s_qn;
    static_assert(LT <= 2048, "a queue entry holds two 11-bit tile indices");
    if constexpr (!DEAD) dead_count = nullptr;
    if (n_live) n_darts = min(n_darts, *n_live);
    const uint32_t lo = blockIdx.x * LT;
    if (lo >= n_darts) return;
    const uint32_t cnt = min((uint32_t)LT, n_darts - lo);
    constexpr int PER = LT / 256;
    uint64_t nk[PER]; uint32_t np[PER], no[PER], nd[PER], succ0[PER], frm[PER];
    if (threadIdx.x == 0) { s_new_count = 0; s_dead_n = 0; s_qn = 0; }
    if (threadIdx.x < kFrameWin) s_fcnt[threadIdx.x] = 0;
    if (dead_count) { for (uint32_t i4 = threadIdx.x; i4 < LT / 4; i4 += 256) reinterpret_cast<uint32_t*>(s_dead)[i4] = 0u; }
    uint32_t sfire = 0;
    uint32_t ecand = 0, epix = 0;
    uint64_t recs[PER];
#pragma unroll
    for (int u = 0; u < PER; u++) {
        const uint32_t d = lo + min(threadIdx.x + u * 256u, cnt - 1u);
        recs[u] = d_rec[d];
        succ0[u] = d_succ[d];
    }
#pragma unroll
    for (int u = 0; u < PER; u++) {
        const uint32_t i = threadIdx.x + u * 256;
        const uint64_t rec = recs[u];
        const uint32_t info = rec_info(rec);
        const uint32_t ek = event_key(rec, W);
        frm[u] = rec_frame(rec);
        nk[u] = ((uint64_t)ek << 32) | (lo + i); np[u] = (succ0[u] - lo) < cnt ? succ0[u] : lo + (uint32_t)LT + i; no[u] = 0; nd[u] = 1;
        if (i < cnt) s_win[i] = Win{nk[u], np[u], 1u << 16};
        if (dead_count && ek != kNoKey) {
            if (static_fire(rec)) sfire |= 1u << u;
            else {
                const uint32_t P = pdart_mask(rec_F(rec));
                ecand |= 1u << u;
                epix |= ((uint32_t)__popc(P & ((1u << (info & 7u)) - 1u)) | ((uint32_t)(__popc(P) - 1) << 2)) << (4 * u);
            }
        }
    }
    if (threadIdx.x == 0) s_f0 = frm[0];
    lds_barrier();
    if (dead_count && sfire) {
#pragma unroll
        for (int u = 0; u < PER; u++)
            if (sfire & (1u << u)) s_dead[threadIdx.x + u * 256] = 2;
    }
    const uint32_t f0 = frame_entries ? s_f0 : 0u;
    uint32_t my_slot[PER];
    uint32_t direct = 0;
#pragma unroll
    for (int u = 0; u < PER; u++) {
        const uint32_t i = threadIdx.x + u * 256;
        my_slot[u] = kNone;
        if (i >= cnt) continue;
        const uint32_t s0 = succ0[u];
        if ((s0 - lo) >= cnt) {
            if (frame_entries) {
                const uint32_t f = frm[u];
                if (f - f0 < kFrameWin) my_slot[u] = atomicAdd(&s_fcnt[f - f0], 1u);
                else {
                    my_slot[u] = frame_base[f] + atomicAdd(&frame_entries[f], 1u);
                    direct |= 1u << u;
                }
            } else my_slot[u] = atomicAdd(&s_new_count, 1u);
        }
    }
    lds_barrier();
    uint32_t slot_a = 0, slot_b = 0;
    if (frame_entries) {
        if (threadIdx.x < kFrameWin && s_fcnt[threadIdx.x]) {
            slot_a = frame_base[f0 + threadIdx.x];
            slot_b = atomicAdd(&frame_entries[f0 + threadIdx.x], s_fcnt[threadIdx.x]);
        }
    } else if (threadIdx.x == 0) {
        slot_a = (blockIdx.x & (kEntryShards - 1)) * ecap;
        if (s_new_count) slot_b = atomicAdd(&entry_count[blockIdx.x & (kEntryShards - 1)], s_new_count);
    }
    constexpr int kLocalRounds = LT == 4096 ? 12 : (LT == 2048 ? 11 : (LT == 1024 ? 10 : 9));
    const int n_rounds = dbg == 0 ? kLocalRounds : (dbg < 0 ? 0 : dbg);
    const bool early = frame_entries == nullptr;
    uint32_t done = 0;
    for (int round = 0; round < n_rounds; round++) {
        uint32_t upd = 0;
#pragma unroll
        for (int u = 0; u < PER; u++) {
            const uint32_t i = threadIdx.x + u * 256;
            if (i < cnt && !((done >> u) & 1u)) {
                const uint32_t t = np[u] - lo;
                if (t < cnt) {
                    const Win w = s_win[t];
                    if (early && w.key == nk[u]) done |= 1u << u;
                    if (w.key < nk[u]) { nk[u] = w.key; no[u] = nd[u] + (w.offdist & 0xFFFFu); }
                    nd[u] += w.offdist >> 16;
                    np[u] = w.ptr;
                    upd |= 1u << u;
                }
            }
        }
        lds_barrier();
#pragma unroll
        for (int u = 0; u < PER; u++) {
            const uint32_t i = threadIdx.x + u * 256;
            if (upd & (1u << u)) s_win[i] = Win{nk[u], np[u], no[u] | (nd[u] << 16)};
        }
        if (round == n_rounds - 1) {
            if (frame_entries) { if (threadIdx.x < kFrameWin) s_fbase[threadIdx.x] = slot_a + slot_b; }
            else if (threadIdx.x == 0) s_new_base = slot_a + slot_b;
        }
        lds_barrier();
    }
    if (n_rounds <= 0) {
        if (frame_entries) { if (threadIdx.x < kFrameWin) s_fbase[threadIdx.x] = slot_a + slot_b; }
        else if (threadIdx.x == 0) s_new_base = slot_a + slot_b;
        lds_barrier();
    }
    if (dead_count) {
#pragma unroll
        for (int u = 0; u < PER; u++) {
            const uint32_t i = threadIdx.x + u * 256;
            const uint32_t sl = succ0[u] - lo;
            const bool push = i < cnt && ((sfire | ecand) & (1u << u)) && (uint32_t)nk[u] == lo + i && (np[u] - lo) < cnt
                              && sl < cnt && sl != i;
            const unsigned long long m = __ballot(push);
            if (m == 0ull) continue;
            uint32_t base = 0;
            if ((threadIdx.x & 63) == (uint32_t)(__ffsll((long long)m) - 1)) base = atomicAdd(&s_qn, (uint32_t)__popcll(m));
            base = __shfl(base, __ffsll((long long)m) - 1);
            const uint32_t slot = base + (uint32_t)__popcll(m & ((1ull << (threadIdx.x & 63)) - 1ull));
            if (push && slot < kQCap) s_q[slot] = i | (sl << 11) | (((epix >> (4 * u)) & 15u) << 22) | (((sfire >> u) & 1u) << 26);
        }
        lds_barrier();
        const uint32_t nq = min(s_qn, kQCap);
        uint32_t my_dead = 0;
        for (uint32_t k = threadIdx.x; k < nq; k += 256) {
            const uint32_t e = s_q[k], i = e & 2047u, sl = (e >> 11) & 2047u;
            const Win wi = s_win[i], ws = s_win[sl];
            if ((uint32_t)ws.key != lo + i) continue;
            const uint32_t n = (ws.offdist & 0xFFFFu) + 1u;
            if (n >= 5u && (uint64_t)n * n >= 8ull * min_edge_length) continue;
            if (!((e >> 26) & 1u)) {
                const uint32_t pi = (e >> 22) & 15u, rank = pi & 3u, others = pi >> 2, first = i - rank;
                if (rank > i || first + others >= cnt) continue;
                const uint32_t ek = (uint32_t)(wi.key >> 32), w2q = ek & ~1u;
                Win wj[4];
#pragma unroll
                for (uint32_t j = 0; j < 4; j++) wj[j] = s_win[first + min(j, others)];
                bool witness = false, closed = true, wfires = true;
#pragma unroll
                for (uint32_t j = 0; j < 4; j++) {
                    const uint32_t lj = (uint32_t)wj[j].key - lo;
                    const bool in_tile = (wj[j].ptr - lo) < cnt, before = (uint32_t)(wj[j].key >> 32) < w2q;
                    if (in_tile && before && lj < cnt && (s_dead[lj] & 2u)) witness = true;
                    closed = closed && in_tile;
                    wfires = wfires && !before;
                }
                const bool is_e = (ek & 1u) != 0u;
                if (!((is_e && witness) || (trust_natural && closed && (is_e ? !wfires : wfires)))) continue;
            }
            s_dead[i] |= 1; my_dead++;
        }
        if (my_dead) atomicAdd(&s_dead_n, my_dead);
        lds_barrier();
        if (threadIdx.x == 0 && s_dead_n) atomicAdd(&dead_count[blockIdx.x & 15u], s_dead_n);
    }
    uint32_t* s_slot = reinterpret_cast<uint32_t*>(s_win);
#pragma unroll
    for (int u = 0; u < PER; u++)
        if (my_slot[u] != kNone) {
            const uint32_t slot = (direct & (1u << u)) ? my_slot[u] : (frame_entries ? s_fbase[frm[u] - f0] : s_new_base) + my_slot[u];
            s_slot[threadIdx.x + u * 256] = slot;
            entry_list[slot] = succ0[u];
        }
    lds_barrier();
    uint32_t lmask = 0;
#pragma unroll
    for (int u = 0; u < PER; u++) {
        const uint32_t i = threadIdx.x + u * 256;
        if (i >= cnt) continue;
        const uint32_t e = np[u];
        const bool frozen = (e - lo) >= cnt;
        const uint32_t li = (uint32_t)nk[u] - lo;
        const bool dead = dead_count != nullptr && !frozen && li < cnt && (s_dead[li] & 1u) != 0;
        const bool event = (uint32_t)(nk[u] >> 32) != kNoKey;
        fin[lo + i] = frozen ? pend_pack(s_slot[(e - lo - (uint32_t)LT) & (uint32_t)(LT - 1)], nd[u], no[u], (uint32_t)nk[u])
                             : FinState{(uint32_t)nk[u], no[u] | (event ? kFinEvent : 0u) | (dead ? kFinDead : 0u)};
        if (!frozen && (uint32_t)nk[u] == lo + i && event && !dead) lmask |= 1u << u;
    }
    if (leader_list) {
        __shared__ uint32_t s_lw[4];
        __shared__ uint32_t s_lbase;
        uint32_t total;
        const uint32_t excl = block_excl_scan_256((uint32_t)__popc(lmask), s_lw, &total);
        if (total) {
            const uint32_t shard = blockIdx.x & (kLeaderShards - 1);
            if (threadIdx.x == 0) s_lbase = atomicAdd(&leader_count[shard], total);
            __syncthreads();
            uint32_t slot = s_lbase + excl;
            while (lmask) {
                const int u = __ffs(lmask) - 1;
                lmask &= lmask - 1;
                leader_list[(size_t)shard * leader_cap + slot++] = lo + threadIdx.x + (uint32_t)u * 256u;
            }
        }
    }
}

constexpr uint32_t kEntryLdsCap = 2048;
__global__ __launch_bounds__(256) void k_entry_frame(const uint32_t* __restrict__ entry_list, const uint32_t* __restrict__ frame_entries,
                                                     const uint32_t* __restrict__ frame_base, const FinState* __restrict__ fin,
                                                     const uint64_t* __restrict__ d_rec, int W,
                                                     EntryState* __restrict__ es, DeviceCounters* __restrict__ ctr,
                                                     uint32_t* __restrict__ leader_list ,
                                                     unsigned int* __restrict__ leader_count , uint32_t leader_cap) {
    struct __attribute__((aligned(16))) Rec { uint64_t key; uint32_t ptr; uint32_t off; };
    __shared__ Rec s_rec[kEntryLdsCap];
    __shared__ uint32_t s_dist[kEntryLdsCap];
    const uint32_t f = blockIdx.x;
    const uint32_t cnt = frame_entries[f], base = frame_base[f];
    if (cnt == 0) return;
    if (cnt > kEntryLdsCap) { if (threadIdx.x == 0) ctr->entry_overflow = 1u; return; }
    constexpr int PER = kEntryLdsCap / 256;
    uint64_t nk[PER]; uint32_t np[PER], no[PER], nd[PER];
    uint32_t m0[PER];
    constexpr int EB = 4;
    static_assert(PER % EB == 0, "whole batches");
#pragma unroll
    for (int u0 = 0; u0 < PER; u0 += EB) {
        if ((uint32_t)u0 * 256u >= cnt) break;
        uint32_t e[EB];
        FinState l[EB];
        uint64_t mr[EB];
#pragma unroll
        for (int u = 0; u < EB; u++) e[u] = entry_list[base + min(threadIdx.x + 256u * (uint32_t)(u0 + u), cnt - 1u)];
#pragma unroll
        for (int u = 0; u < EB; u++) l[u] = fin[e[u]];
#pragma unroll
        for (int u = 0; u < EB; u++) mr[u] = d_rec[entry_min_dart(e[u], l[u])];
#pragma unroll
        for (int u = 0; u < EB; u++) asm volatile("" : "+v"(mr[u]), "+v"(l[u].leader), "+v"(l[u].w));
#pragma unroll
        for (int u = 0; u < EB; u++) {
            const uint32_t i = threadIdx.x + 256u * (uint32_t)(u0 + u);
            const EntryState s0 = entry_start(e[u], l[u], mr[u], W, base + i);
            nk[u0 + u] = s0.key; no[u0 + u] = s0.off; nd[u0 + u] = s0.dist; np[u0 + u] = s0.ptr - base; m0[u0 + u] = (uint32_t)s0.key;
            if (i < cnt) { s_rec[i] = Rec{nk[u0 + u], np[u0 + u], no[u0 + u]}; s_dist[i] = nd[u0 + u]; }
        }
    }
    __syncthreads();
    for (int round = 0; round < 12; round++) {
        int changed = 0;
#pragma unroll
        for (int u = 0; u < PER; u++) {
            const uint32_t i = threadIdx.x + u * 256;
            if (i < cnt) {
                const uint32_t t = np[u] < cnt ? np[u] : i;
                const Rec w = s_rec[t];
                const uint32_t wd = s_dist[t];
                if (w.key < nk[u]) { nk[u] = w.key; no[u] = nd[u] + w.off; changed = 1; }
                nd[u] += wd;
                np[u] = w.ptr;
            }
        }
        const int any = __syncthreads_or(changed);
#pragma unroll
        for (int u = 0; u < PER; u++) {
            const uint32_t i = threadIdx.x + u * 256;
            if (i < cnt) { s_rec[i] = Rec{nk[u], np[u], no[u]}; s_dist[i] = nd[u]; }
        }
        __syncthreads();
        if (!any) break;
    }
#pragma unroll
    for (int u = 0; u < PER; u++) {
        const uint32_t i = threadIdx.x + u * 256;
        if (i < cnt) {
            EntryState o;
            o.key = nk[u]; o.ptr = base + np[u]; o.off = no[u]; o.dist = nd[u]; o.pad = 0;
            es[base + i] = o;
        }
// ... 520 lines not shown
            best = group_max_u64<G>(best);
            const unsigned long long num = best >> 30;
            if (num == 0) continue;
            const uint32_t index = ~(uint32_t)best & 0x3FFFFFFFu;
            const double dn = (double)num, den = (double)((long long)la * la + (long long)lb * lb);
            const double lhs = dn * dn, rhs = eps * eps * den;
            bool far;
            if (lhs > rhs * (1.0 + 1e-9)) far = true;
            else if (lhs < rhs * (1.0 - 1e-9)) far = false;
            else far = dn / sqrt(den) > eps;
            if (far) {
                if (splits == 3) { reject = true; break; }
                kept[splits++] = index;
                seg_a[nseg] = a; seg_b[nseg] = index; nseg++;
                seg_a[nseg] = index; seg_b[nseg] = b; nseg++;
            }
        }
        if (reject || splits != 3) continue;
        if (lane != 0) continue;
        uint32_t k0 = kept[0], k1 = kept[1], k2 = kept[2], t;
        if (k0 > k1) { t = k0; k0 = k1; k1 = t; }
        if (k1 > k2) { t = k1; k1 = k2; k2 = t; }
        if (k0 > k1) { t = k0; k0 = k1; k1 = t; }
        const uint32_t idx[4] = {0u, k0, k1, k2};
        int q[8], hq[8];
        for (int i = 0; i < 4; i++) { const uint32_t p = P[idx[i]]; q[2 * i] = p & 0xFFFF; q[2 * i + 1] = p >> 16; }
        if (!hull4(q, hq)) continue;
        uint32_t cmin = min_edge_length + 1u;
        for (int i = 0; i < 4; i++) {
            const int j = (i + 1) & 3;
            const int dx = hq[2 * i] - hq[2 * j], dy = hq[2 * i + 1] - hq[2 * j + 1];
            const uint32_t d2 = (uint32_t)(dx * dx + dy * dy);
            cmin = d2 < cmin ? d2 : cmin;
        }
        if (cmin < min_edge_length) continue;
        enforce_clockwise(hq);
        const uint32_t fl = r.frame - first_frame;
        const uint32_t slot = atomicAdd(&cand_count[fl], 1u);
        if (slot >= max_cand) { atomicOr(err_flags, kErrCandTable); continue; }
        CandRec cr;
        cr.start_key = r.start_key;
        for (int i = 0; i < 8; i++) cr.xy[i] = (uint16_t)hq[i];
        cands[(size_t)fl * max_cand + slot] = cr;
    }
}

__global__ __launch_bounds__(256) void k_contour_quads(uint32_t blocks64, const ContourRec* __restrict__ contours, const DeviceCounters* __restrict__ ctr,
                                                       uint32_t max_contours, const uint32_t* __restrict__ points, double eps_factor,
                                                       uint32_t min_edge_length, uint32_t first_frame, uint32_t max_cand,
                                                       CandRec* __restrict__ cands, uint32_t* __restrict__ cand_count,
                                                       unsigned int* __restrict__ err_flags, int coords14) {
    if (blockIdx.x < blocks64)
        contour_quads_body<64>(blockIdx.x, blocks64, contours, ctr, max_contours, points, eps_factor, min_edge_length, first_frame, max_cand, cands,
                               cand_count, err_flags, coords14 != 0);
    else
        contour_quads_body<16>(blockIdx.x - blocks64, gridDim.x - blocks64, contours, ctr, max_contours, points, eps_factor, min_edge_length,
                               first_frame, max_cand, cands, cand_count, err_flags, coords14 != 0);
}

__global__ void k_unpack_bits(const uint64_t* __restrict__ bits, int W, int H, uint8_t* __restrict__ out) {
    const int x = blockIdx.x * blockDim.x + threadIdx.x, y = blockIdx.y;
    if (x >= W) return;
    const int wpr = (int)words_per_row((uint32_t)W);
    out[(size_t)y * W + x] = ((bits[(size_t)y * wpr + (x >> 6)] >> (x & 63)) & 1ull) ? 255 : 0;
}

constexpr int kFinBlocks = 1536;
static inline int blocks_for(uint64_t n, int per_block, int cap) {
    uint64_t b = (n + per_block - 1) / per_block;
    if (b < 1) b = 1;
    if (b > (uint64_t)cap) b = cap;
    return (int)b;
}

__global__ __launch_bounds__(256) void k_zero(uint4* __restrict__ p, uint32_t n16) {
    for (uint32_t i = blockIdx.x * blockDim.x + threadIdx.x; i < n16; i += gridDim.x * blockDim.x) p[i] = make_uint4(0u, 0u, 0u, 0u);
}
hipError_t launch_zero(hipStream_t st, void* p, size_t bytes ) {
    const uint32_t n16 = (uint32_t)(bytes / 16);
    hipLaunchKernelGGL(k_zero, dim3(blocks_for(n16, 256, 256)), dim3(256), 0, st, reinterpret_cast<uint4*>(p), n16);
    return hipGetLastError();
}

size_t tile_mask_offset_bytes(uint32_t W, uint32_t H, uint32_t n_frames);
size_t tile_darts_bytes(uint32_t W, uint32_t H, uint32_t n_frames) { return tile_mask_offset_bytes(W, H, n_frames) + (size_t)dart_tiles(W, H) * n_frames * kCountHalves * 8; }
size_t tile_off_offset(uint32_t W, uint32_t H, uint32_t n_frames) { return (size_t)dart_tiles(W, H) * n_frames; }
size_t tile_mask_offset_bytes(uint32_t W, uint32_t H, uint32_t n_frames) { return ((size_t)dart_tiles(W, H) * n_frames * 4 * (1 + kCountHalves) + 7) & ~(size_t)7; }

hipError_t launch_dart_count(hipStream_t st, const uint64_t* bits, int W, int H, uint32_t first_frame, uint32_t n_frames,
                             unsigned long long* frame_darts, uint32_t* tile_darts, uint64_t plan_cap, uint32_t* frame_base, uint32_t* plan,
                             void* zero_p, size_t zero_bytes ) {
    const uint32_t tiles_x = dart_tiles_x((uint32_t)W), tiles_y = ((uint32_t)H + kTileRows - 1) / kTileRows;
    const uint32_t wpr = words_per_row((uint32_t)W);
    uint32_t* h1 = tile_darts + (size_t)tiles_x * tiles_y * n_frames * 2;
    unsigned long long* tmask = reinterpret_cast<unsigned long long*>(reinterpret_cast<uint8_t*>(tile_darts) + tile_mask_offset_bytes((uint32_t)W, (uint32_t)H, n_frames));
    if (wpr <= 30)
        hipLaunchKernelGGL(k_dart_count<32>, dim3((tiles_y + 1) / 2, n_frames, kCountHalves), dim3(64), 0, st, bits, W, H, first_frame, frame_darts, tile_darts, h1, tmask);
    else
        hipLaunchKernelGGL(k_dart_count<64>, dim3(((wpr + kCountLanes - 1) / kCountLanes) * tiles_y, n_frames, kCountHalves), dim3(64), 0, st, bits, W, H, first_frame,
                           frame_darts, tile_darts, h1, tmask);
    hipLaunchKernelGGL(k_tile_scan, dim3(n_frames + (plan ? 1u : 0u)), dim3(256), 0, st, tile_darts, h1, tiles_x * tiles_y, first_frame,
                       tile_darts + (size_t)tiles_x * tiles_y * n_frames, n_frames, frame_darts, (unsigned long long)plan_cap, frame_base, plan,
                       reinterpret_cast<uint4*>(zero_p), (uint32_t)(zero_bytes / 16));
    return hipGetLastError();
}

hipError_t launch_dart_build(hipStream_t st, const uint64_t* bits, int W, int H, uint32_t first_frame, uint32_t n_frames,
                             const uint32_t* frame_base, const uint32_t* tile_off, uint32_t* pix_base, const uint32_t* tile_darts, uint64_t* d_rec,
                             uint32_t* d_succ, uint32_t n_darts, const uint32_t* n_live, int dbg, const unsigned long long* tile_mask) {
    const uint32_t tiles = dart_tiles((uint32_t)W, (uint32_t)H);
    hipLaunchKernelGGL(k_dart_assign, dim3((tiles * n_frames + 7u) / 8u * 8u), dim3(256), 0, st, bits, W, H, first_frame, frame_base, tile_off,
                       pix_base, tile_darts, d_rec, d_succ, n_live, dbg, tile_mask, tiles, n_frames);
    if (dbg && dbg != 5) return hipGetLastError();
    hipLaunchKernelGGL(k_dart_link, dim3(blocks_for(n_darts, 256, 4096)), dim3(256), 0, st, W, H, first_frame, pix_base, bits, d_rec, d_succ, n_darts, n_live);
    return hipGetLastError();
}

size_t entry_state_bytes() { return sizeof(EntryState); }
bool finalize_inline(bool frame_entries, bool trust_natural) { return frame_entries && trust_natural; }
size_t fin_state_bytes() { return sizeof(FinState); }
size_t entry_slots(uint32_t n_darts) { return (size_t)entry_shard_cap(n_darts) * kEntryShards; }
size_t leader_list_bytes(uint32_t n_darts) { return (size_t)leader_shard_cap(n_darts) * kLeaderShards * 4; }

hipError_t launch_rank_cycles(hipStream_t st, uint32_t n_darts, int W, const uint64_t* d_rec, const uint32_t* d_succ,
                              uint32_t* entry_list,
                              unsigned int* entry_count, void* es_a, void* es_b, void* fin8 , uint32_t* leader_list,
                              unsigned int* leader_count, int max_rounds, DeviceCounters* ctr, const uint32_t* n_live, int dbg,
                              const uint32_t* frame_base, uint32_t* frame_entries , uint32_t n_frames,
                              int phase ,
                              uint32_t min_edge_length, unsigned int* dead_count ,
                              int trust_natural ) {
    const uint32_t ecap = entry_shard_cap(n_darts);
    FinState* fin = reinterpret_cast<FinState*>(fin8);
    const bool no_finalize = finalize_inline(frame_entries != nullptr, trust_natural != 0) && dbg == 0;
    uint32_t* const ll = no_finalize ? leader_list : nullptr;
    const uint32_t lcap = leader_shard_cap(n_darts);
    if (phase != 2) {
        if (frame_entries && !dead_count)
            hipLaunchKernelGGL((k_local_contract<kLTFrame, false>), dim3((n_darts + kLTFrame - 1) / kLTFrame), dim3(256), 0, st, n_darts, W, d_rec, d_succ, fin,
                               entry_list, entry_count, ecap, frame_base, frame_entries, n_live, dbg, min_edge_length, dead_count, trust_natural,
                               ll, leader_count, lcap);
        else if (frame_entries)
            hipLaunchKernelGGL((k_local_contract<kLTFrame, true>), dim3((n_darts + kLTFrame - 1) / kLTFrame), dim3(256), 0, st, n_darts, W, d_rec, d_succ, fin,
                               entry_list, entry_count, ecap, frame_base, frame_entries, n_live, dbg, min_edge_length, dead_count, trust_natural,
                               ll, leader_count, lcap);
        else
            hipLaunchKernelGGL((k_local_contract<kLT, true>), dim3((n_darts + kLT - 1) / kLT), dim3(256), 0, st, n_darts, W, d_rec, d_succ, fin,
                               entry_list, entry_count, ecap, frame_base, frame_entries, n_live, dbg, min_edge_length, dead_count, trust_natural,
                               ll, leader_count, lcap);
    }
    if (dbg || phase == 1) return hipGetLastError();
    EntryState* a = reinterpret_cast<EntryState*>(es_a);
    EntryState* b = reinterpret_cast<EntryState*>(es_b);
    if (frame_entries) {
        hipLaunchKernelGGL(k_entry_frame, dim3(n_frames), dim3(256), 0, st, entry_list, frame_entries, frame_base, fin, d_rec, W, a, ctr,
                           ll, leader_count, lcap);
        if (no_finalize) return hipGetLastError();
        const int fin_blocks = std::max(blocks_for(n_darts, 256, kFinBlocks), (int)(((uint64_t)n_darts + 256ull * 32 - 1) / (256ull * 32)));
        hipLaunchKernelGGL(k_jump_finalize, dim3(fin_blocks), dim3(256), 0, st, n_darts, a, fin,
                           leader_list, leader_count, leader_shard_cap(n_darts), n_live, ctr);
        return hipGetLastError();
    }
    const dim3 grid(blocks_for(n_darts / 16 + 1, 256, 1024)), block(256);
    hipLaunchKernelGGL(k_entry_init, grid, block, 0, st, entry_list, entry_count, fin, d_rec, W, a, ecap);
    for (int r = 0; r < max_rounds; r++) {
        hipLaunchKernelGGL(k_entry_jump, grid, block, 0, st, a, b, entry_count, ecap, r, ctr);
        EntryState* t = a; a = b; b = t;
    }
    const int fin_blocks = std::max(blocks_for(n_darts, 256, kFinBlocks), (int)(((uint64_t)n_darts + 256ull * 32 - 1) / (256ull * 32)));
    hipLaunchKernelGGL(k_jump_finalize, dim3(fin_blocks), block, 0, st, n_darts, a, fin,
                       leader_list, leader_count, leader_shard_cap(n_darts), n_live, ctr);
    return hipGetLastError();
}

hipError_t launch_resolve(hipStream_t st, const void* fin8, uint32_t n_darts, int W, const uint64_t* d_rec, const uint32_t* leader_list,
                          const unsigned int* leader_count, uint64_t* t_cur, uint64_t* t_next, DeviceCounters* ctr, int max_iters,
                          const uint32_t* n_live) {
    const FinState* fin = reinterpret_cast<const FinState*>(fin8);
    if (max_iters <= 0) return hipSuccess;
    const dim3 grid(blocks_for(n_darts, 256, 4096)), block(256);
    hipLaunchKernelGGL(k_resolve_fast, dim3(blocks_for(n_darts / 16 + 1, 256, 1024)), block, 0, st, fin, leader_list, leader_count,
                       leader_shard_cap(n_darts), W, d_rec, t_cur, ctr);
    hipLaunchKernelGGL(k_resolve_init, grid, block, 0, st, fin, d_rec, W, n_darts, t_cur, t_next, ctr, n_live);
    for (int it = 0; it < max_iters; it++) {
        hipLaunchKernelGGL(k_resolve_eval, grid, block, 0, st, fin, n_darts, W, d_rec, t_cur, t_next, it, ctr, n_live);
        hipLaunchKernelGGL(k_resolve_commit, grid, block, 0, st, fin, n_darts, t_cur, t_next, it, it == max_iters - 1 ? 1 : 0, ctr, n_live);
    }
    return hipGetLastError();
}

hipError_t launch_select_scatter(hipStream_t st, const void* fin8, uint32_t n_darts, const uint32_t* leader_list,
                                 const unsigned int* leader_count, const uint32_t* d_succ, const uint64_t* t_cur,
                                 const uint32_t* frame_base, uint32_t n_frames, uint32_t first_frame, uint32_t min_edge_length,
                                 double eps_factor, double image_diag, ContourRec* contours, uint32_t* cyc_start_off,
                                 uint32_t max_contours, uint64_t max_points, DeviceCounters* ctr, const uint64_t* d_rec, uint32_t* points,
// ... 35 lines not shown
```

aruco3_amd/csrc/k_decode.hip:

```cpp

#include "a3_common.h"
#include "a3_ippe.h"

namespace a3 {

__device__ __forceinline__ float perimeter4(const uint16_t* q) {
    float p = 0.0f;
#pragma unroll
    for (int i = 0; i < 4; i++) {
        const int j = (i + 1) & 3;
        const float dx = (float)q[2 * i] - (float)q[2 * j];
        const float dy = (float)q[2 * i + 1] - (float)q[2 * j + 1];
        p += sqrtf((dx * dx) + (dy * dy));
    }
    return p;
}

struct __attribute__((aligned(8))) ProjRec { float inv[9]; int ok; };
__device__ bool solve_projection(const float* from, float S, float* inv_out);

constexpr uint32_t kFrameCandLds = 6144;
constexpr int kFcWaves = 1;
template <bool BIG>
__global__ __launch_bounds__(64, kFcWaves) void k_frame_candidates(const CandRec* __restrict__ cands, const uint32_t* __restrict__ cand_count,
// ... 245 lines not shown
typedef const uint32_t __attribute__((address_space(1)))* a3_gptr;

template <typename OffT>
__device__ __forceinline__ void sample_issue(TapLoad& tl, a3_gptr base4, uint32_t mis, OffT row_stride, OffT wide_limit, bool tiny,
                                             uint32_t bpp, uint32_t w, uint32_t h, float x, float y, bool valid) {
    const float left = floorf(x), right = left + 1.0f, top = floorf(y), bottom = top + 1.0f;
    tl.rw = x - left; tl.bw = y - top;
    const bool inside = valid & !((left < 0.0f) | (right >= (float)w) | (top < 0.0f) | (bottom >= (float)h));
    const uint32_t lc = sat_u32(left), tc = sat_u32(top), bc = sat_u32(bottom);
    const uint32_t l = inside ? lc : 0u, t = inside ? tc : 0u, b = inside ? bc : 0u;
    tl.l = l; tl.t = t;
    OffT ot, ob;
    if constexpr (sizeof(OffT) == 4) {
        const uint32_t xl = __umul24(bpp, l);
        ot = __umul24(t, (uint32_t)row_stride) + xl; ob = __umul24(b, (uint32_t)row_stride) + xl;
    } else {
        ot = (OffT)t * row_stride + (OffT)(bpp * l); ob = (OffT)b * row_stride + (OffT)(bpp * l);
    }
    const bool wide = inside & !tiny & (ob <= wide_limit);
    tl.mode = inside ? (wide ? 1 : 2) : 0;
    const OffT at = (wide ? ot : (OffT)0) + (OffT)mis, ab = (wide ? ob : (OffT)0) + (OffT)mis;
    const a3_gptr qt = base4 + (at >> 2), qb = base4 + (ab >> 2);
    tl.top[0] = qt[0]; tl.top[1] = qt[1]; tl.top[2] = qt[2];
    tl.bot[0] = qb[0]; tl.bot[1] = qb[1]; tl.bot[2] = qb[2];
    tl.sh = ((uint32_t)(at & 3u) * 8u) | (((uint32_t)(ab & 3u) * 8u) << 8);
}

__device__ __forceinline__ void pair_from(const uint32_t d[3], uint32_t sh, int fmt, uint32_t bpp, float* g0, float* g1) {
    const uint32_t w0 = __builtin_amdgcn_alignbit(d[1], d[0], sh), w1 = __builtin_amdgcn_alignbit(d[2], d[1], sh);
    if (bpp == 1u) { *g0 = (float)(w0 & 0xFFu); *g1 = (float)((w0 >> 8) & 0xFFu); return; }
    const bool bgr = fmt == A3_FMT_BGRA8;
    const uint32_t px1 = bpp == 3u ? ((w0 >> 24) | (w1 << 8)) : w1;
    *g0 = (float)luma_px(w0, bgr);
    *g1 = (float)luma_px(px1, bgr);
}

__device__ __forceinline__ uint8_t sample_finish(const TapLoad& tl, const uint8_t* __restrict__ img, size_t row_stride, int fmt, uint32_t bpp) {
    float a, b, c, d;
    pair_from(tl.top, tl.sh & 0xFFu, fmt, bpp, &a, &b);
    pair_from(tl.bot, tl.sh >> 8, fmt, bpp, &c, &d);
    if (tl.mode == 2) {
        const uint8_t* rt = img + (size_t)tl.t * row_stride;
        const uint8_t* rb = rt + row_stride;
        a = grey_tap(rt, tl.l, fmt); b = grey_tap(rt, tl.l + 1u, fmt); c = grey_tap(rb, tl.l, fmt); d = grey_tap(rb, tl.l + 1u, fmt);
    }
    const uint8_t tv = clamp_u8((1.0f - tl.rw) * a + tl.rw * b);
    const uint8_t bv = clamp_u8((1.0f - tl.rw) * c + tl.rw * d);
    const uint8_t v = clamp_u8((1.0f - tl.bw) * (float)tv + tl.bw * (float)bv);
    return tl.mode == 0 ? (uint8_t)0 : v;
}

__device__ __forceinline__ float triangle_kernel(float x) { return fabsf(x) < 1.0f ? 1.0f - fabsf(x) : 0.0f; }

__device__ uint32_t resize_weights(uint32_t in_len, uint32_t out_len, uint32_t o, float* ws, uint32_t* count) {
    const float ratio = (float)in_len / (float)out_len;
    const float sratio = ratio < 1.0f ? 1.0f : ratio;
    const float src_support = 1.0f * sratio;
    float input = ((float)o + 0.5f) * ratio;
    long long left = (long long)floorf(input - src_support);
    left = left < 0 ? 0 : (left > (long long)in_len - 1 ? (long long)in_len - 1 : left);
    long long right = (long long)ceilf(input + src_support);
    right = right < left + 1 ? left + 1 : (right > (long long)in_len ? (long long)in_len : right);
    input = input - 0.5f;
    float sum = 0.0f;
    uint32_t n = 0;
    for (long long i = left; i < right; i++) {
        const float w = triangle_kernel(((float)i - input) / sratio);
        ws[n++] = w;
        sum += w;
    }
    for (uint32_t i = 0; i < n; i++) ws[i] /= sum;
    *count = n;
    return (uint32_t)left;
}


constexpr size_t kWeightTableBytes = 16384;
__global__ void k_weight_table(uint32_t S, uint32_t n, uint32_t max_taps, float* __restrict__ wtab) {
    if (threadIdx.x >= n) return;
    float* row = wtab + (size_t)threadIdx.x * (max_taps + 2);
    uint32_t cnt;
    const uint32_t left = resize_weights(S, n, threadIdx.x, row + 2, &cnt);
    row[0] = __uint_as_float(left); row[1] = __uint_as_float(cnt);
}
__global__ __launch_bounds__(64, kFcWaves) void k_projection(const uint16_t* __restrict__ fin_xy, const uint32_t* __restrict__ work,
                                                   const unsigned int* __restrict__ work_count, uint32_t S, ProjRec* __restrict__ proj) {
    const uint32_t n_work = *work_count;
    for (uint32_t wi = blockIdx.x * blockDim.x + threadIdx.x; wi < n_work; wi += gridDim.x * blockDim.x) {
        const uint32_t slot = work[wi];
        const uint16_t* q = fin_xy + (size_t)slot * 8;
        float from[8];
        for (int i = 0; i < 8; i++) from[i] = (float)q[i];
        ProjRec r;
        r.ok = solve_projection(from, (float)S, r.inv) ? 1 : 0;
        proj[wi] = r;
    }
}

__device__ __forceinline__ void rotated_source(uint32_t r, uint32_t n, uint32_t y, uint32_t x, uint32_t* sy, uint32_t* sx) {
    if (r == 0) { *sy = y; *sx = x; }
    else if (r == 1) { *sy = x; *sx = n - 1 - y; }
    else if (r == 2) { *sy = n - 1 - y; *sx = n - 1 - x; }
    else { *sy = n - 1 - x; *sx = y; }
}

constexpr int kDecodeKU = 2;
constexpr int kDecodeThreads = 256;
constexpr int kDecodeWaves = 5;
constexpr int kDecodeDB = 8;
#define A3_DPP_STEPS(STEP) STEP(0x111, 0xF) STEP(0x112, 0xF) STEP(0x114, 0xF) STEP(0x118, 0xF) STEP(0x142, 0xA) STEP(0x143, 0xC)
__device__ __forceinline__ uint32_t wave_incl_add(uint32_t v) {
#define A3_S(CTRL, RM) v += (uint32_t)__builtin_amdgcn_update_dpp(0, (int)v, CTRL, RM, 0xF, false);
    A3_DPP_STEPS(A3_S)
#undef A3_S
    return v;
}
__device__ __forceinline__ unsigned long long wave_min_u64_to63(unsigned long long v) {
#define A3_S(CTRL, RM)                                                                                                  \
    {                                                                                                                    \
        const uint32_t lo_ = (uint32_t)__builtin_amdgcn_update_dpp(-1, (int)(uint32_t)v, CTRL, RM, 0xF, false);           \
        const uint32_t hi_ = (uint32_t)__builtin_amdgcn_update_dpp(-1, (int)(uint32_t)(v >> 32), CTRL, RM, 0xF, false);    \
        const unsigned long long o_ = ((unsigned long long)hi_ << 32) | lo_;                                             \
        v = o_ < v ? o_ : v;                                                                                             \
    }
    A3_DPP_STEPS(A3_S)
#undef A3_S
    return v;
}
__device__ __forceinline__ void wave_best_var_to63(double& var, int& best_t) {
#define A3_S(CTRL, RM)                                                                                                  \
    {                                                                                                                    \
        const unsigned long long vb_ = (unsigned long long)__double_as_longlong(var);                                    \
        const uint32_t lo_ = (uint32_t)__builtin_amdgcn_update_dpp(0, (int)(uint32_t)vb_, CTRL, RM, 0xF, false);           \
        const uint32_t hi_ = (uint32_t)__builtin_amdgcn_update_dpp((int)0xBFF00000u, (int)(uint32_t)(vb_ >> 32), CTRL, RM, 0xF, false); \
        const int ot_ = __builtin_amdgcn_update_dpp(0x7FFFFFFF, best_t, CTRL, RM, 0xF, false);                             \
        const double ov_ = __longlong_as_double((long long)(((unsigned long long)hi_ << 32) | lo_));                     \
        if (ov_ > var || (ov_ == var && ot_ < best_t)) { var = ov_; best_t = ot_; }                                      \
    }
    A3_DPP_STEPS(A3_S)
#undef A3_S
}

__device__ __forceinline__ void compact_frame_wave(uint32_t f, int lane, const DecodeOut* __restrict__ outs, const uint16_t* __restrict__ fin_xy,
                                                   const uint32_t* __restrict__ fin_count, uint32_t n_frames, uint32_t max_cand,
                                                   a3_marker* __restrict__ markers, uint32_t marker_cap, const uint32_t* __restrict__ per_frame,
                                                   unsigned int* __restrict__ marker_total, unsigned int* __restrict__ err_flags,
                                                   const uint32_t* __restrict__ cand_count, unsigned int* __restrict__ cand_pre_total) {
    uint32_t base = 0;
    for (uint32_t g = lane; g < f; g += 64) base += per_frame[g];
    for (int o = 32; o > 0; o >>= 1) base += __shfl_xor(base, o);
    if (f + 1 == n_frames && lane == 0) *marker_total = base + per_frame[f];
    if (f + 1 == n_frames) {
        uint32_t pre = 0, most = 0;
        for (uint32_t g = lane; g < n_frames; g += 64) { pre += min(cand_count[g], max_cand); most = max(most, cand_count[g]); }
        for (int o = 32; o > 0; o >>= 1) { pre += __shfl_xor(pre, o); most = max(most, (uint32_t)__shfl_xor(most, o)); }
        if (lane == 0) { *cand_pre_total = pre; cand_pre_total[3] = most; }
    }
    const uint32_t c = fin_count[f];
    uint32_t pos = base;
    for (uint32_t k0 = 0; k0 < c; k0 += 64) {
        const uint32_t k = k0 + lane;
        DecodeOut o;
        o.valid = 0;
        if (k < c) o = outs[(size_t)f * max_cand + k];
        const unsigned long long m = __ballot(o.valid != 0);
        if (o.valid) {
            const uint32_t p = pos + (uint32_t)__popcll(m & ((1ull << lane) - 1ull));
            if (p < marker_cap) {
                a3_marker mk;
                mk.frame = f;
                mk.id = o.id;
                mk.code = o.code;
                const uint16_t* q = fin_xy + ((size_t)f * max_cand + k) * 8;
                for (int i = 0; i < 4; i++) {
                    const int s2 = (i + o.rotation) & 3;
                    mk.corners[2 * i] = q[2 * s2];
                    mk.corners[2 * i + 1] = q[2 * s2 + 1];
                }
                mk.hamming_distance = o.hamming;
                mk.rotation = o.rotation;
                mk.candidate_index = (uint16_t)k;
                markers[p] = mk;
            } else atomicOr(err_flags, kErrMarkerCap);
        }
        pos += (uint32_t)__popcll(m);
    }
}

template <int NT, int PT>
__global__ __launch_bounds__(NT, kDecodeWaves) void k_decode(PixelSrc src, int W, int H, uint32_t first_frame,
                                                const uint16_t* __restrict__ fin_xy, const uint32_t* __restrict__ work,
                                                const unsigned int* __restrict__ work_count, uint32_t max_cand, uint32_t S, uint32_t n,
                                                uint32_t max_taps, const uint64_t* __restrict__ dict, uint32_t n_codes, uint32_t tau,
                                                int filter, const ProjRec* __restrict__ proj, const float* __restrict__ wtab, DecodeOut* __restrict__ outs,
                                                uint8_t* __restrict__ patches , uint32_t patch_cap, uint32_t* __restrict__ per_frame , int dbg) {
    extern __shared__ __attribute__((aligned(16))) uint8_t smem[];
    uint8_t* s_patch = smem;
    size_t o = ((size_t)S * S + 15) & ~(size_t)15;
    float* s_tmp = reinterpret_cast<float*>(smem + o); o += (size_t)n * S * 4;
    float* s_w = reinterpret_cast<float*>(smem + o); o += (size_t)n * max_taps * 4;
    uint32_t* s_left = reinterpret_cast<uint32_t*>(smem + o); o += (size_t)n * 4;
    uint32_t* s_cnt = reinterpret_cast<uint32_t*>(smem + o); o += (size_t)n * 4;
    uint8_t* s_bits = smem + o;
    __shared__ uint32_t s_hist[256];
    __shared__ float s_inv[9];
    __shared__ int s_ok, s_have;
    __shared__ uint32_t s_otsu;
    __shared__ uint64_t s_codes[4];
    __shared__ unsigned long long s_best[NT / 64][4];
    constexpr int NW = NT / 64;
    __shared__ uint32_t s_scan_w[NW], s_scan_s[NW];
    __shared__ double s_var[NW];
    __shared__ int s_vt[NW];

    const int tid = threadIdx.x;
    const uint32_t n_work = *work_count;
    for (uint32_t wi = blockIdx.x; wi < n_work; wi += gridDim.x) {
        const uint32_t slot = work[wi];
        const uint32_t fl = slot / max_cand;
        const uint8_t* img = src.base + (size_t)(first_frame + fl) * src.frame_stride;
        __syncthreads();
        if (tid < 9) s_inv[tid] = proj[wi].inv[tid];
        if (tid == 9) s_ok = proj[wi].ok;
        for (int i = tid; i < 256; i += NT) s_hist[i] = 0;
        __syncthreads();
        const bool ok = s_ok != 0;
        const uint32_t pw = ok ? S : 1u, ph = pw;
        if (ok) {
            for (uint32_t i = tid; i < n * (max_taps + 2); i += NT) {
                const uint32_t oi = i / (max_taps + 2), k = i - oi * (max_taps + 2);
                const float v = wtab[i];
                if (k == 0) s_left[oi] = __float_as_uint(v);
                else if (k == 1) s_cnt[oi] = __float_as_uint(v);
                else if (k - 2 < __float_as_uint(wtab[(size_t)oi * (max_taps + 2) + 1])) s_w[(size_t)oi * max_taps + (k - 2)] = v;
            }
        } else if (tid < (int)n) {
            const uint32_t oi = tid;
            uint32_t cnt;
            s_left[oi] = resize_weights(pw, n, oi, s_w + (size_t)oi * max_taps, &cnt);
            s_cnt[oi] = cnt;
        }
        if (ok && dbg == 1) {
            for (uint32_t i = tid; i < S * S; i += NT) { s_patch[i] = (uint8_t)(i * 7u); atomicAdd(&s_hist[(i * 7u) & 255u], 1u); }
        } else if (ok) {
            const float t0 = s_inv[0], t1 = s_inv[1], t2 = s_inv[2], t3 = s_inv[3], t4 = s_inv[4], t5 = s_inv[5], t6 = s_inv[6],
                        t7 = s_inv[7], t8 = s_inv[8];
            constexpr int kU = kDecodeKU;
            const uint32_t bpp = (src.fmt == A3_FMT_RGB8) ? 3u : ((src.fmt == A3_FMT_RGBA8 || src.fmt == A3_FMT_BGRA8) ? 4u : 1u);
            const unsigned long long frame_bytes = (unsigned long long)(H - 1) * src.row_stride + (unsigned long long)W * bpp;
            const bool tiny = frame_bytes < 16ull, off32 = frame_bytes < 0xFFFFFFE0ull && src.row_stride < (1ull << 24);
            const uintptr_t img_u = reinterpret_cast<uintptr_t>(img);
            const uint32_t mis = tiny ? 0u : (uint32_t)(img_u & 3u);
            const a3_gptr base4 = reinterpret_cast<a3_gptr>(tiny ? reinterpret_cast<uintptr_t>(wtab) : img_u - mis);
            const uint32_t nbx = (S + 7u) / 8u, n_slots = nbx * nbx * 64u;
            const uint32_t Mb = 65536u / nbx + 1u;
            auto slot_xy = [&](uint32_t slot, uint32_t* x, uint32_t* y) -> bool {
                const uint32_t blk = slot >> 6, l = slot & 63u, by = __umul24(min(blk, 1023u), Mb) >> 16, bx = blk - __umul24(by, nbx);
                *x = bx * 8u + (l & 7u); *y = by * 8u + (l >> 3);
                return slot < n_slots && *x < S && *y < S;
            };
            for (uint32_t i0 = tid; i0 < n_slots; i0 += NT * kU) {
                TapLoad tl[kU];
#pragma unroll
                for (int u = 0; u < kU; u++) {
                    uint32_t x, y;
                    const bool valid = slot_xy(i0 + (uint32_t)NT * u, &x, &y);
                    const float fx = (float)x, fy = (float)y;
                    const float d = t6 * fx + t7 * fy + t8;
                    const float px = (t0 * fx + t1 * fy + t2) / d;
                    const float py = (t3 * fx + t4 * fy + t5) / d;
                    if (off32) sample_issue<uint32_t>(tl[u], base4, mis, (uint32_t)src.row_stride, (uint32_t)(frame_bytes - 12ull), tiny, bpp, (uint32_t)W, (uint32_t)H, px, py, valid);
                    else sample_issue<unsigned long long>(tl[u], base4, mis, src.row_stride, frame_bytes - 12ull, tiny, bpp, (uint32_t)W, (uint32_t)H, px, py, valid);
                }
#pragma unroll
                for (int u = 0; u < kU; u++) {
                    uint32_t x, y;
                    if (slot_xy(i0 + (uint32_t)NT * u, &x, &y)) {
                        const uint8_t v = sample_finish(tl[u], img, (size_t)src.row_stride, src.fmt, bpp);
                        s_patch[__umul24(y, S) + x] = v;
                        atomicAdd(&s_hist[v], 1u);
                    }
                }
            }
        } else if (tid == 0) {
            s_patch[0] = 0;
            s_hist[0] = 1;
        }
        __syncthreads();
        if (dbg == 2) continue;
        static_assert(PT == 64 || PT == NT, "the stages after the sampling run on one wave or on all");
        constexpr int NWP = PT / 64;
#define POST_SYNC() { if constexpr (PT == NT) __syncthreads(); else { __builtin_amdgcn_fence(__ATOMIC_ACQ_REL, "wavefront"); __builtin_amdgcn_wave_barrier(); } }
        if (PT == NT || tid < PT) {
            const bool keep_patch = patches != nullptr && wi < patch_cap;
            if (keep_patch) {
                uint8_t* dst = patches + (size_t)wi * S * S;
                for (uint32_t i = tid; i < S * S; i += PT) dst[i] = ok ? s_patch[i] : 0;
            }
            {
                constexpr int B = 256 / PT;
                uint32_t cw[B], cs[B];
                uint32_t rw = 0, rs = 0;
    #pragma unroll
                for (int k = 0; k < B; k++) {
                    const uint32_t t = (uint32_t)tid * B + k, hcnt = s_hist[t];
                    rw += hcnt; rs += t * hcnt;
                    cw[k] = rw; cs[k] = rs;
                }
                uint32_t bw = wave_incl_add(rw), bs = wave_incl_add(rs);
                if ((tid & 63) == 63) { s_scan_w[tid >> 6] = bw; s_scan_s[tid >> 6] = bs; }
                POST_SYNC();
                uint32_t total_sum_u = 0;
                for (int w = 0; w < NWP; w++) {
                    if (w < (tid >> 6)) { bw += s_scan_w[w]; bs += s_scan_s[w]; }
                    total_sum_u += s_scan_s[w];
                }
                const uint32_t before_w = bw - rw, before_s = bs - rs;
                const uint32_t total_weight = pw * ph;
                const double total_pixel_sum = (double)total_sum_u;
                double var = -1.0;
                int best_t = tid * B;
    #pragma unroll
                for (int k = 0; k < B; k++) {
                    const uint32_t bwk = before_w + cw[k], bsk = before_s + cs[k];
                    const uint32_t fw = total_weight - bwk;
                    if (bwk != 0 && fw != 0) {
                        const double background_pixel_sum = (double)bsk;
                        const double foreground_pixel_sum = total_pixel_sum - background_pixel_sum;
                        const double background_mean = background_pixel_sum / (double)bwk;
// ... 283 lines not shown
    out[2 * i + 1] = p2;
}

__global__ void k_find_nearest(const uint64_t* __restrict__ dict, uint32_t n_codes, const uint64_t* __restrict__ bits, uint32_t n,
                               uint32_t* __restrict__ idx, uint8_t* __restrict__ dist) {
    const int lane = threadIdx.x & 63;
    const uint32_t qi = (blockIdx.x * blockDim.x + threadIdx.x) >> 6;
    if (qi >= n) return;
    const uint64_t b = bits[qi];
    unsigned long long best = ~0ull;
    for (uint32_t i = lane; i < n_codes; i += 64) {
        const unsigned long long k = ((unsigned long long)__popcll(dict[i] ^ b) << 32) | i;
        best = k < best ? k : best;
    }
    for (int o = 32; o > 0; o >>= 1) {
        const unsigned long long other = __shfl_xor(best, o);
        best = other < best ? other : best;
    }
    if (lane == 0) {
        idx[qi] = n_codes ? (uint32_t)best : 0u;
        dist[qi] = n_codes ? (uint8_t)(best >> 32) : 0xFF;
    }
}

__global__ void k_calc_tau(const uint64_t* __restrict__ dict, uint32_t n_codes, unsigned int* __restrict__ tau) {
    unsigned int best = 255;
    for (uint32_t i = blockIdx.x * blockDim.x + threadIdx.x; i < n_codes; i += gridDim.x * blockDim.x) {
        const uint64_t c = dict[i];
        for (uint32_t j = i + 1; j < n_codes; j++) {
            const unsigned int d = __popcll(c ^ dict[j]);
            best = d < best ? d : best;
        }
    }
    for (int o = 32; o > 0; o >>= 1) { const unsigned int other = __shfl_xor(best, o); best = other < best ? other : best; }
    if ((threadIdx.x & 63) == 0) atomicMin(tau, best);
}

__global__ void k_selftest_ieee(const double* __restrict__ a, const double* __restrict__ b, uint32_t n, double* __restrict__ sq,
                                double* __restrict__ dv, float* __restrict__ sqf, float* __restrict__ dvf) {
    const uint32_t i = blockIdx.x * blockDim.x + threadIdx.x;
    if (i >= n) return;
    sq[i] = sqrt(a[i]);
    dv[i] = a[i] / b[i];
    sqf[i] = sqrtf((float)a[i]);
    dvf[i] = (float)a[i] / (float)b[i];
}

size_t decode_lds_bytes(uint32_t S, uint32_t n, uint32_t max_taps) {
    size_t o = ((size_t)S * S + 15) & ~(size_t)15;
    o += (size_t)n * S * 4 + (size_t)n * max_taps * 4 + (size_t)n * 8 + (size_t)n * n;
    return (o + 15) & ~(size_t)15;
}

hipError_t launch_frame_candidates(hipStream_t st, const CandRec* cands, const uint32_t* cand_count, uint32_t n_frames, uint32_t max_cand,
                                   float min_distance, uint16_t* pre_xy, uint16_t* fin_xy, uint32_t* fin_count, uint32_t* work,
                                   unsigned int* work_count, uint32_t S, void* proj, float* big_scratch ) {
    const bool big = max_cand > kFrameCandLds;
    if (big && !big_scratch) return hipErrorInvalidValue;
    const size_t lds = big ? (size_t)max_cand + 16 : (size_t)max_cand * 21 + 16;
    if (lds > 48 * 1024) {
        const hipError_t e = hipFuncSetAttribute(big ? reinterpret_cast<const void*>(k_frame_candidates<true>) : reinterpret_cast<const void*>(k_frame_candidates<false>),
                                                 hipFuncAttributeMaxDynamicSharedMemorySize, (int)lds);
        if (e != hipSuccess) return e;
    }
    if (big)
        hipLaunchKernelGGL(k_frame_candidates<true>, dim3(n_frames), dim3(64), lds, st, cands, cand_count, max_cand, min_distance, pre_xy, fin_xy,
                           fin_count, work, work_count, S, reinterpret_cast<ProjRec*>(proj), big_scratch);
    else
        hipLaunchKernelGGL(k_frame_candidates<false>, dim3(n_frames), dim3(64), lds, st, cands, cand_count, max_cand, min_distance, pre_xy, fin_xy,
                           fin_count, work, work_count, S, reinterpret_cast<ProjRec*>(proj), nullptr);
    return hipGetLastError();
}
uint32_t frame_cand_lds_slots() { return kFrameCandLds; }

size_t proj_rec_bytes() { return sizeof(ProjRec); }
size_t weight_table_bytes() { return kWeightTableBytes; }
hipError_t launch_weight_table(hipStream_t st, uint32_t S, uint32_t n, uint32_t max_taps, float* wtab) {
    if ((size_t)n * (max_taps + 2) * 4 > kWeightTableBytes || n > 64) return hipErrorInvalidValue;
    hipLaunchKernelGGL(k_weight_table, dim3(1), dim3(64), 0, st, S, n, max_taps, wtab);
    return hipGetLastError();
}

hipError_t launch_decode(hipStream_t st, PixelSrc src, int W, int H, uint32_t first_frame, const uint16_t* fin_xy, const uint32_t* work,
                         const unsigned int* work_count, uint32_t max_cand, uint32_t S, uint32_t n, uint32_t max_taps, const uint64_t* dict,
                         uint32_t n_codes, uint32_t tau, int filter, void* proj, const float* wtab, void* outs, uint8_t* patches, uint32_t patch_cap, uint32_t* per_frame, int grid_blocks, int dbg, int few) {
    ProjRec* recs = reinterpret_cast<ProjRec*>(proj);
    if (dbg > 0 || dbg == -1000) hipLaunchKernelGGL(k_projection, dim3(256), dim3(64), 0, st, fin_xy, work, work_count, S, recs);
    const int d = dbg == -1000 ? 0 : (dbg < 0 ? -dbg : dbg);
    if (few)
        hipLaunchKernelGGL((k_decode<256, 256>), dim3(grid_blocks), dim3(256), decode_lds_bytes(S, n, max_taps), st, src, W, H, first_frame, fin_xy, work, work_count,
                           max_cand, S, n, max_taps, dict, n_codes, tau, filter, recs, wtab, reinterpret_cast<DecodeOut*>(outs), patches, patch_cap, per_frame, d);
    else
        hipLaunchKernelGGL((k_decode<kDecodeThreads, 64>), dim3(grid_blocks), dim3(kDecodeThreads), decode_lds_bytes(S, n, max_taps), st, src, W, H, first_frame, fin_xy, work,
                           work_count, max_cand, S, n, max_taps, dict, n_codes, tau, filter, recs, wtab, reinterpret_cast<DecodeOut*>(outs), patches, patch_cap,
                           per_frame, d);
    return hipGetLastError();
}

size_t decode_out_bytes() { return sizeof(DecodeOut); }

hipError_t launch_compact_markers(hipStream_t st, const void* outs, const uint16_t* fin_xy, const uint32_t* fin_count, uint32_t n_frames,
                                  uint32_t first_frame, uint32_t max_cand, a3_marker* markers, uint32_t marker_cap, uint32_t* per_frame,
                                  unsigned int* marker_total, unsigned int* err_flags, const uint32_t* cand_count, unsigned int* cand_pre_total) {
    if (first_frame == 0 && n_frames <= kCompactParMax)
        hipLaunchKernelGGL(k_compact_markers_par, dim3((n_frames + 3) / 4), dim3(256), 0, st, reinterpret_cast<const DecodeOut*>(outs), fin_xy, fin_count,
                           n_frames, max_cand, markers, marker_cap, per_frame, marker_total, err_flags, cand_count, cand_pre_total);
    else
        hipLaunchKernelGGL(k_compact_markers, dim3(1), dim3(256), 0, st, reinterpret_cast<const DecodeOut*>(outs), fin_xy, fin_count, n_frames,
                           first_frame, max_cand, markers, marker_cap, per_frame, marker_total, err_flags, cand_count, cand_pre_total);
    return hipGetLastError();
}

hipError_t launch_pack_detections(hipStream_t st, const a3_marker* markers, const a3_pose* poses, const uint32_t* per_frame, uint32_t n_frames,
                                  uint32_t first_frame_global, uint32_t maxm, void* dst, unsigned int* overflow) {
    hipLaunchKernelGGL(k_pack_detections, dim3((n_frames + 3) / 4), dim3(256), 0, st, markers, poses, per_frame, n_frames, first_frame_global, maxm,
                       reinterpret_cast<uint32_t*>(dst), overflow);
    return hipGetLastError();
}

hipError_t launch_debug_rotate_bits(hipStream_t st, const uint8_t* in, uint32_t n, uint32_t r, uint8_t* out) {
    hipLaunchKernelGGL(k_debug_rotate_bits, dim3(1), dim3(256), 0, st, in, n, r, out);
    return hipGetLastError();
}

hipError_t launch_pose(hipStream_t st, const uint32_t* corners, uint32_t corner_stride, const float* norm_pts, uint32_t n,
                       const unsigned int* n_dev, int mode, float marker_size_mm, float iw, float ih, float fx, float fy, float cx, float cy,
                       a3_pose* out) {
    hipLaunchKernelGGL(k_pose, dim3((n + 63) / 64), dim3(64), 0, st, corners, corner_stride, norm_pts, n, n_dev, mode, marker_size_mm, iw, ih,
                       fx, fy, cx, cy, out);
    return hipGetLastError();
}

hipError_t launch_find_nearest(hipStream_t st, const uint64_t* dict, uint32_t n_codes, const uint64_t* bits, uint32_t n, uint32_t* idx,
                               uint8_t* dist) {
    hipLaunchKernelGGL(k_find_nearest, dim3((n * 64 + 255) / 256), dim3(256), 0, st, dict, n_codes, bits, n, idx, dist);
    return hipGetLastError();
}

hipError_t launch_calc_tau(hipStream_t st, const uint64_t* dict, uint32_t n_codes, unsigned int* tau) {
    hipLaunchKernelGGL(k_calc_tau, dim3(64), dim3(256), 0, st, dict, n_codes, tau);
    return hipGetLastError();
}

hipError_t launch_selftest(hipStream_t st, const double* a, const double* b, uint32_t n, double* sq, double* dv, float* sqf, float* dvf) {
    hipLaunchKernelGGL(k_selftest_ieee, dim3((n + 255) / 256), dim3(256), 0, st, a, b, n, sq, dv, sqf, dvf);
    return hipGetLastError();
}

}
```

Before: 383,100.

## Compact non-empty tiles into a list and loop dart-assign over it

The tile scan now emits a compacted list of non-empty tiles with their dart offsets plus a per-frame count, in place of a dense offset array. Dart-assign launches about half as many workgroups per frame, each walking the list with a stride. Register tile loads and scalar prefetches are issued early to hide latency. Decode now reads the inverse homography and ok flag straight into scalar registers instead of going through LDS, drops a per-entry tap-count check by zero-padding the weight table, and clamps its work index so loads can be issued before the bounds check. The risks are more serial work per workgroup when many tiles are active, and an extra scan in the tile scan kernel.

```diff
diff --git a/aruco3_amd/csrc/a3_api.hip b/aruco3_amd/csrc/a3_api.hip
--- a/aruco3_amd/csrc/a3_api.hip
+++ b/aruco3_amd/csrc/a3_api.hip
@@ -17,10 +17,8 @@
 bool threshold_writes_grey_plane(uint32_t radius, const uint8_t* pixels, size_t row_stride, size_t frame_stride, int W);
 hipError_t launch_dart_count(hipStream_t, const uint64_t*, int, int, uint32_t, uint32_t, unsigned long long*, uint32_t*, uint64_t, uint32_t*, uint32_t*, void*, size_t);
 size_t tile_darts_bytes(uint32_t W, uint32_t H, uint32_t n_frames);
-size_t tile_off_offset(uint32_t W, uint32_t H, uint32_t n_frames);
-size_t tile_mask_offset_bytes(uint32_t W, uint32_t H, uint32_t n_frames);
-hipError_t launch_dart_build(hipStream_t, const uint64_t*, int, int, uint32_t, uint32_t, const uint32_t*, const uint32_t*, uint32_t*, const uint32_t*,
-                             uint64_t*, uint32_t*, uint32_t, const uint32_t*, int, const unsigned long long*);
+hipError_t launch_dart_build(hipStream_t, const uint64_t*, int, int, uint32_t, uint32_t, const uint32_t*, uint32_t*, const uint32_t*, uint32_t, bool,
+                             uint64_t*, uint32_t*, uint32_t, const uint32_t*, int);
 hipError_t launch_zero(hipStream_t, void*, size_t);
 size_t entry_state_bytes();
 bool finalize_inline(bool frame_entries, bool trust_natural);
@@ -47,7 +45,7 @@
 size_t proj_rec_bytes();
 size_t weight_table_bytes();
 hipError_t launch_weight_table(hipStream_t, uint32_t, uint32_t, uint32_t, float*);
-hipError_t launch_decode(hipStream_t, PixelSrc, int, int, uint32_t, const uint16_t*, const uint32_t*, const unsigned int*, uint32_t,
+hipError_t launch_decode(hipStream_t, PixelSrc, int, int, uint32_t, const uint16_t*, const uint32_t*, const unsigned int*, uint32_t, uint32_t,
                          uint32_t, uint32_t, uint32_t, const uint64_t*, uint32_t, uint32_t, int, void*, const float*, void*, uint8_t*, uint32_t, uint32_t*, int, int, int);
 hipError_t launch_compact_markers(hipStream_t, const void*, const uint16_t*, const uint32_t*, uint32_t, uint32_t, uint32_t, a3_marker*,
                                   uint32_t, uint32_t*, unsigned int*, unsigned int*, const uint32_t*, unsigned int*);
@@ -416,7 +414,7 @@
                                    ctx->work.as<uint32_t>(), d_work_count, S, ctx->proj.p, ctx->cand_big.as<float>()));
     const int few = b.n <= 64u ? 1 : 0;
     A3_HIP(launch_decode(st, b.src, (int)b.W, (int)b.H, 0, ctx->fin_xy.as<uint16_t>(), ctx->work.as<uint32_t>(), d_work_count,
-                         b.max_cand, S, ctx->mark_size, S, ctx->dict.as<uint64_t>(), ctx->n_codes, ctx->tau, ctx->cfg.filter_high_bit_errors,
+                         b.n, b.max_cand, S, ctx->mark_size, S, ctx->dict.as<uint64_t>(), ctx->n_codes, ctx->tau, ctx->cfg.filter_high_bit_errors,
                          ctx->proj.p, ctx->wtab.as<float>(), ctx->outs.p, b.taps ? ctx->patches.as<uint8_t>() : nullptr, b.patch_cap, ctx->per_frame,
                          (int)std::min<uint32_t>(4096u, b.n * 128u) , 0,
                          few));
@@ -776,10 +774,8 @@
             A3_HIP(hipMemsetAsync(d_leader_count, 0, 4 * 32, st));
             A3_HIP(hipMemsetAsync(ctx->frame_cursor, 0, (size_t)c.count * 4, st));
         }
-        const uint32_t* tile_off = ctx->tile_darts.as<uint32_t>() + tile_off_offset(W, H, n);
-        A3_HIP(launch_dart_build(st, d_bin, (int)W, (int)H, c.first, c.count, fb, tile_off, ctx->pix_base.as<uint32_t>(),
-                                 ctx->tile_darts.as<uint32_t>(), ctx->d_xy.as<uint64_t>(), ctx->d_succ.as<uint32_t>(), nd, n_live, 0,
-                                 reinterpret_cast<const unsigned long long*>(ctx->tile_darts.as<uint8_t>() + tile_mask_offset_bytes(W, H, n))));
+        A3_HIP(launch_dart_build(st, d_bin, (int)W, (int)H, c.first, c.count, fb, ctx->pix_base.as<uint32_t>(), ctx->tile_darts.as<uint32_t>(), n,
+                                 ctx->entry_global_ttl > 0, ctx->d_xy.as<uint64_t>(), ctx->d_succ.as<uint32_t>(), nd, n_live, 0));
         int rounds = 1;
         while ((1ull << rounds) < (uint64_t)c.max_frame_darts && rounds < 31) rounds++;
         rounds += 1;
@@ -1489,10 +1485,8 @@
                                      ctx->tile_darts.as<uint32_t>(), 0, nullptr, nullptr, nullptr, 0));
         } else if (kernel == 1) {
             A3_HIP(launch_dart_build(st, ctx->bin.as<uint64_t>(), (int)ctx->W, (int)ctx->H, 0, ctx->dbg_frames, ctx->frame_base.as<uint32_t>(),
-                                     ctx->tile_darts.as<uint32_t>() + tile_off_offset(ctx->W, ctx->H, ctx->frames), ctx->pix_base.as<uint32_t>(),
-                                     ctx->tile_darts.as<uint32_t>(), ctx->d_xy.as<uint64_t>(),
-                                     ctx->d_succ.as<uint32_t>(), ctx->dbg_nd, nullptr, dbg ? dbg : 5,
-                                     reinterpret_cast<const unsigned long long*>(ctx->tile_darts.as<uint8_t>() + tile_mask_offset_bytes(ctx->W, ctx->H, ctx->frames))));
+                                     ctx->pix_base.as<uint32_t>(), ctx->tile_darts.as<uint32_t>(), ctx->frames, ctx->entry_global_ttl > 0,
+                                     ctx->d_xy.as<uint64_t>(), ctx->d_succ.as<uint32_t>(), ctx->dbg_nd, nullptr, dbg ? dbg : 5));
         } else if (kernel == 2) {
             A3_HIP(launch_rank_cycles(st, ctx->dbg_nd, (int)ctx->W, ctx->d_xy.as<uint64_t>(), ctx->d_succ.as<uint32_t>(),
                                       ctx->entry_list.as<uint32_t>(),
@@ -1506,7 +1500,7 @@
                 A3_HIP(hipEventRecord(e0, st));
             }
             A3_HIP(launch_decode(st, ctx->dbg_src, (int)ctx->W, (int)ctx->H, 0, ctx->fin_xy.as<uint16_t>(), ctx->work.as<uint32_t>(), ctx->scratch_u32,
-                                 ctx->max_cand, ctx->cfg.homography_sample_size, ctx->mark_size, ctx->cfg.homography_sample_size, ctx->dict.as<uint64_t>(),
+                                 ctx->frames, ctx->max_cand, ctx->cfg.homography_sample_size, ctx->mark_size, ctx->cfg.homography_sample_size, ctx->dict.as<uint64_t>(),
                                  ctx->n_codes, ctx->tau, ctx->cfg.filter_high_bit_errors, ctx->proj.p, ctx->wtab.as<float>(), ctx->outs.p, nullptr, 0u, nullptr, 4096,
                                  dbg == 0 ? -1000 : dbg, ctx->frames <= 64u ? 1 : 0));
         } else return fail(ctx, A3_ERR_INVALID, "kernel: 0 dart_count, 1 dart_assign, 2 local_contract, 3 decode, 4 decode on cold frames");
diff --git a/aruco3_amd/csrc/k_contours.hip b/aruco3_amd/csrc/k_contours.hip
--- a/aruco3_amd/csrc/k_contours.hip
+++ b/aruco3_amd/csrc/k_contours.hip
@@ -23,6 +23,13 @@
     }
 }
 
+__device__ __forceinline__ void lds_barrier() {
+    __builtin_amdgcn_fence(__ATOMIC_RELEASE, "workgroup", "local");
+    __builtin_amdgcn_s_barrier();
+    __builtin_amdgcn_fence(__ATOMIC_ACQUIRE, "workgroup", "local");
+}
+
+template <bool LDS_ONLY = false>
 __device__ __forceinline__ uint32_t block_excl_scan_256(uint32_t v, uint32_t* s_wave, uint32_t* total) {
     const int lane = threadIdx.x & 63, wave = threadIdx.x >> 6;
     uint32_t inc = v;
@@ -35,7 +42,7 @@
     A3_DPP_ADD(0x143, 0xC)
 #undef A3_DPP_ADD
     if (lane == 63) s_wave[wave] = inc;
-    __syncthreads();
+    if constexpr (LDS_ONLY) lds_barrier(); else __syncthreads();
     uint32_t base = 0, tot = 0;
 #pragma unroll
     for (int w = 0; w < 4; w++) {
@@ -51,13 +58,12 @@
 __host__ __device__ inline uint32_t dart_tiles_x(uint32_t W) { return (words_per_row(W) + kTileWords - 1) / kTileWords; }
 __host__ __device__ inline uint32_t dart_tiles(uint32_t W, uint32_t H) { return dart_tiles_x(W) * ((H + kTileRows - 1) / kTileRows); }
 
-__device__ __forceinline__ void tile_stage(const uint64_t* __restrict__ img, int W, int H, uint32_t tile, uint64_t (*s_t)[kTileWords + 2]) {
+constexpr int kStage = (kTileRows + 2) * (kTileWords + 2);
+static_assert(kStage <= 512, "two words per lane");
+__device__ __forceinline__ void tile_load(const uint64_t* __restrict__ img, int W, int H, uint32_t tile, uint64_t v[2]) {
     const int wpr = (int)words_per_row((uint32_t)W);
     const int tx = tile % dart_tiles_x((uint32_t)W), ty = tile / dart_tiles_x((uint32_t)W);
     const int j0 = tx * kTileWords - 1, y0 = ty * kTileRows - 1;
-    constexpr int kStage = (kTileRows + 2) * (kTileWords + 2);
-    static_assert(kStage <= 512, "two words per lane");
-    uint64_t v[2];
 #pragma unroll
     for (int k = 0; k < 2; k++) {
         const int i = min((int)threadIdx.x + 256 * k, kStage - 1);
@@ -66,6 +72,8 @@
         const uint64_t w = img[(size_t)min(max(yy, 0), H - 1) * wpr + min(max(jj, 0), wpr - 1)];
         v[k] = w & (0ull - (uint64_t)(yy >= 0 && yy < H && jj >= 0 && jj < wpr));
     }
+}
+__device__ __forceinline__ void tile_store(const uint64_t v[2], uint64_t (*s_t)[kTileWords + 2]) {
 #pragma unroll
     for (int k = 0; k < 2; k++) {
         const int i = (int)threadIdx.x + 256 * k;
@@ -253,7 +261,7 @@
 }
 
 __global__ __launch_bounds__(256) void k_tile_scan(uint32_t* __restrict__ tile_darts, const uint32_t* __restrict__ tile_darts_h1, uint32_t tiles, uint32_t first_frame,
-                                                   uint32_t* __restrict__ tile_off, uint32_t n_frames,
+                                                   uint2* __restrict__ tile_list, uint32_t* __restrict__ tile_cnt, uint32_t n_frames,
                                                    unsigned long long* __restrict__ frame_darts, unsigned long long cap,
                                                    uint32_t* __restrict__ frame_base, uint32_t* __restrict__ plan,
                                                    uint4* __restrict__ zero_p, uint32_t zero_n16) {
@@ -263,10 +271,10 @@
         plan_frames(frame_darts, n_frames, cap, frame_base, plan);
         return;
     }
-    __shared__ uint32_t s_wave[4];
-    __shared__ uint32_t s_run;
+    __shared__ uint32_t s_wave[4], s_wave_t[4];
+    __shared__ uint32_t s_run, s_run_t;
     const size_t base = (size_t)(first_frame + blockIdx.x) * tiles;
-    if (threadIdx.x == 0) s_run = 0;
+    if (threadIdx.x == 0) { s_run = 0; s_run_t = 0; }
     __syncthreads();
     for (uint32_t t0 = 0; t0 < tiles; t0 += 256) {
         const uint32_t t = t0 + threadIdx.x;
@@ -276,14 +284,15 @@
 #pragma unroll
             for (int z = 1; z < kCountHalves; z++) v += tile_darts_h1[(size_t)(z - 1) * n_frames * tiles + base + t];
         }
-        if (t < tiles) tile_darts[base + t] = v;
-        uint32_t total;
+        uint32_t total, total_t;
         const uint32_t excl = block_excl_scan_256(v, s_wave, &total);
-        if (t < tiles) tile_off[base + t] = s_run + excl;
+        const uint32_t rank = block_excl_scan_256(v ? 1u : 0u, s_wave_t, &total_t);
+        if (v) tile_list[base + s_run_t + rank] = make_uint2(t, s_run + excl);
         __syncthreads();
-        if (threadIdx.x == 0) s_run += total;
+        if (threadIdx.x == 0) { s_run += total; s_run_t += total_t; }
         __syncthreads();
     }
+    if (threadIdx.x == 0) tile_cnt[first_frame + blockIdx.x] = s_run_t;
 }
 
 __device__ __forceinline__ uint32_t row3(uint64_t l, uint64_t c, uint64_t r, int i) {
@@ -336,11 +345,11 @@
 __device__ __forceinline__ int dir_dy(int k) { return (int)((0xA901u >> (2 * k)) & 3u) - 1; }
 
 __global__ __launch_bounds__(256) void k_dart_assign(const uint64_t* __restrict__ bits, int W, int H, uint32_t first_frame,
-                                                     const uint32_t* __restrict__ frame_base, const uint32_t* __restrict__ tile_off,
-                                                     uint32_t* __restrict__ pix_base, const uint32_t* __restrict__ tile_darts,
+                                                     const uint32_t* __restrict__ frame_base, uint32_t* __restrict__ pix_base,
                                                      uint64_t* __restrict__ d_rec, uint32_t* __restrict__ d_succ,
                                                      const uint32_t* __restrict__ n_live, int dbg,
-                                                     const unsigned long long* __restrict__ tile_mask, uint32_t tiles, uint32_t n_frames) {
+                                                     const unsigned long long* __restrict__ tile_mask, uint32_t tiles, uint32_t n_frames,
+                                                     const uint2* __restrict__ tile_list, const uint32_t* __restrict__ tile_cnt, uint32_t wpf) {
     __shared__ uint32_t s_wave[4];
     __shared__ uint64_t s_t[kTileRows + 2][kTileWords + 2];
     __shared__ uint64_t s_nodes[256];
@@ -352,25 +361,40 @@
     __shared__ uint32_t s_multi;
     __shared__ uint16_t s_lut[256];
     const int wpr = (int)words_per_row((uint32_t)W);
-    const uint32_t n_wg = tiles * n_frames, chunk = (n_wg + 7u) >> 3, g = (blockIdx.x & 7u) * chunk + (blockIdx.x >> 3);
+    __shared__ uint32_t s_cnt[256];
+    const uint32_t n_wg = wpf * n_frames, chunk = (n_wg + 7u) >> 3, g = (blockIdx.x & 7u) * chunk + (blockIdx.x >> 3);
     if (g >= n_wg) return;
-    const uint32_t f = g / tiles, tile = g - f * tiles;
-    if (tile_darts[(size_t)(first_frame + f) * tiles + tile] == 0u) return;
-    if (n_live && *n_live == 0u) return;
-    const uint32_t dart0 = frame_base[f] + tile_off[(size_t)(first_frame + f) * tiles + tile];
+    const uint32_t f = g / wpf, wx = g - f * wpf;
+    const size_t fbase = (size_t)(first_frame + f) * tiles;
+    const uint32_t* const live_p = n_live ? n_live : tile_cnt;
+    const uint32_t cnt = tile_cnt[first_frame + f];
+    uint2 ent = tile_list[fbase + wx];
+    const uint32_t dart_f = frame_base[f];
+    const uint32_t live = *live_p;
+    const uint16_t lutv = kPixLut.v[threadIdx.x];
+    asm volatile("" ::"s"(cnt), "s"(ent.x), "s"(ent.y), "s"(dart_f), "s"(live), "v"(lutv));
+    if (wx >= cnt) return;
+    if (n_live && live == 0u) return;
     if (dbg == 1) return;
-    __shared__ uint32_t s_cnt[256];
-    const unsigned long long* tm = tile_mask + ((size_t)(first_frame + f) * tiles + tile) * kCountHalves;
+    const int tiles_x = (int)dart_tiles_x((uint32_t)W);
+    uint32_t* pbf = pix_base + (size_t)f * W * H;
+    s_lut[threadIdx.x] = lutv;
+    for (uint32_t e = wx;;) {
+    const uint32_t tile = ent.x, dart0 = dart_f + ent.y;
+    const unsigned long long* tm = tile_mask + (fbase + tile) * kCountHalves;
     static_assert(kCountHalves == 4 && kTileWords == 4 && kTileRows == 64, "four 64-bit word masks per tile, four word columns of 64 rows");
+    uint64_t tw[2];
+    tile_load(bits + (size_t)(first_frame + f) * wpr * H, W, H, tile, tw);
+    const unsigned long long tm0 = tm[0], tm1 = tm[1], tm2 = tm[2], tm3 = tm[3];
+    asm volatile("" ::"v"(tw[0]), "v"(tw[1]), "s"(tm0), "s"(tm1), "s"(tm2), "s"(tm3));
     unsigned long long cm[4];
 #pragma unroll
     for (int c = 0; c < 4; c++)
-        cm[c] = ((tm[0] >> (16 * c)) & 0xFFFFull) | (((tm[1] >> (16 * c)) & 0xFFFFull) << 16) | (((tm[2] >> (16 * c)) & 0xFFFFull) << 32) | (((tm[3] >> (16 * c)) & 0xFFFFull) << 48);
+        cm[c] = ((tm0 >> (16 * c)) & 0xFFFFull) | (((tm1 >> (16 * c)) & 0xFFFFull) << 16) | (((tm2 >> (16 * c)) & 0xFFFFull) << 32) | (((tm3 >> (16 * c)) & 0xFFFFull) << 48);
     const unsigned long long m0 = cm[0], m1 = cm[1], m2 = cm[2], m3 = cm[3];
-    tile_stage(bits + (size_t)(first_frame + f) * wpr * H, W, H, tile, s_t);
+    tile_store(tw, s_t);
     s_cnt[threadIdx.x] = 0;
     s_mark[threadIdx.x] = 0; s_mark[256 + threadIdx.x] = 0;
-    s_lut[threadIdx.x] = kPixLut.v[threadIdx.x];
     if (threadIdx.x == 0) s_multi = 0;
     __syncthreads();
     const uint32_t a0 = (uint32_t)__popcll(m0), a1 = a0 + (uint32_t)__popcll(m1), a2 = a1 + (uint32_t)__popcll(m2), n_act = a2 + (uint32_t)__popcll(m3);
@@ -415,8 +439,7 @@
     if (dbg == 2) return;
     __syncthreads();
     if (dbg == 3) return;
-    const int tx = tile % dart_tiles_x((uint32_t)W), ty = tile / dart_tiles_x((uint32_t)W);
-    uint32_t* pbf = pix_base + (size_t)f * W * H;
+    const int tx = (int)tile % tiles_x, ty = (int)tile / tiles_x;
     const bool single = __builtin_amdgcn_readfirstlane((int)s_multi) == 0;
     for (uint32_t n = threadIdx.x; n < total_n; n += 256) {
         const uint32_t seg = n >> 6;
@@ -465,6 +488,11 @@
             cur++;
         }
     }
+    e += wpf;
+    if (e >= cnt) break;
+    ent = tile_list[fbase + e];
+    lds_barrier();
+    }
 }
 
 __device__ __forceinline__ uint32_t pixel_F(const uint64_t* __restrict__ img, int wpr, int H, int x, int y) {
@@ -597,12 +625,6 @@
 __device__ __forceinline__ uint32_t entry_min_dart(uint32_t e, FinState s) { return is_pending(s) ? pend_min(s, e) : s.leader; }
 __device__ __forceinline__ FinState fin_final(FinState s, uint32_t d, const EntryState* __restrict__ es) {
     return (es != nullptr && is_pending(s)) ? resolve_pending(s, d, es[pend_slot(s)]) : s;
-}
-
-__device__ __forceinline__ void lds_barrier() {
-    __builtin_amdgcn_fence(__ATOMIC_RELEASE, "workgroup", "local");
-    __builtin_amdgcn_s_barrier();
-    __builtin_amdgcn_fence(__ATOMIC_ACQUIRE, "workgroup", "local");
 }
 
 __device__ __forceinline__ bool static_fire(uint64_t rec) {
@@ -635,10 +657,7 @@
     __shared__ uint32_t s_qn;
     static_assert(LT <= 2048, "a queue entry holds two 11-bit tile indices");
     if constexpr (!DEAD) dead_count = nullptr;
-    if (n_live) n_darts = min(n_darts, *n_live);
     const uint32_t lo = blockIdx.x * LT;
-    if (lo >= n_darts) return;
-    const uint32_t cnt = min((uint32_t)LT, n_darts - lo);
     constexpr int PER = LT / 256;
     uint64_t nk[PER]; uint32_t np[PER], no[PER], nd[PER], succ0[PER], frm[PER];
     if (threadIdx.x == 0) { s_new_count = 0; s_dead_n = 0; s_qn = 0; }
@@ -647,12 +666,27 @@
     uint32_t sfire = 0;
     uint32_t ecand = 0, epix = 0;
     uint64_t recs[PER];
+    if constexpr (DEAD) {
+        if (n_live) n_darts = min(n_darts, *n_live);
+        if (lo >= n_darts) return;
+    }
+    const uint32_t last = n_darts - 1u - lo;
+    if constexpr (!DEAD) asm volatile("" ::"s"(last), "s"(d_rec), "s"(d_succ));
+    const uint32_t* const live_p = n_live ? n_live : frame_base;
+    const uint32_t live = DEAD ? 0u : *live_p;
 #pragma unroll
     for (int u = 0; u < PER; u++) {
-        const uint32_t d = lo + min(threadIdx.x + u * 256u, cnt - 1u);
+        const uint32_t d = lo + min(threadIdx.x + u * 256u, DEAD ? min((uint32_t)LT, n_darts - lo) - 1u : last);
         recs[u] = d_rec[d];
         succ0[u] = d_succ[d];
     }
+    if constexpr (!DEAD) {
+        static_assert(DEAD || PER == 4, "the statement below names every load");
+        asm volatile("" ::"s"(live), "v"(recs[0]), "v"(recs[1]), "v"(recs[2]), "v"(recs[3]), "v"(succ0[0]), "v"(succ0[1]), "v"(succ0[2]), "v"(succ0[3]));
+        if (n_live) n_darts = min(n_darts, live);
+        if (lo >= n_darts) return;
+    }
+    const uint32_t cnt = min((uint32_t)LT, n_darts - lo);
 #pragma unroll
     for (int u = 0; u < PER; u++) {
         const uint32_t i = threadIdx.x + u * 256;
@@ -805,29 +839,76 @@
             entry_list[slot] = succ0[u];
         }
     lds_barrier();
-    uint32_t lmask = 0;
-#pragma unroll
-    for (int u = 0; u < PER; u++) {
+    auto final_of = [&](int u, bool* leads) -> FinState {
         const uint32_t i = threadIdx.x + u * 256;
-        if (i >= cnt) continue;
         const uint32_t e = np[u];
         const bool frozen = (e - lo) >= cnt;
         const uint32_t li = (uint32_t)nk[u] - lo;
         const bool dead = dead_count != nullptr && !frozen && li < cnt && (s_dead[li] & 1u) != 0;
         const bool event = (uint32_t)(nk[u] >> 32) != kNoKey;
-        fin[lo + i] = frozen ? pend_pack(s_slot[(e - lo - (uint32_t)LT) & (uint32_t)(LT - 1)], nd[u], no[u], (uint32_t)nk[u])
-                             : FinState{(uint32_t)nk[u], no[u] | (event ? kFinEvent : 0u) | (dead ? kFinDead : 0u)};
-        if (!frozen && (uint32_t)nk[u] == lo + i && event && !dead) lmask |= 1u << u;
-    }
-    if (leader_list) {
-        __shared__ uint32_t s_lw[4];
-        __shared__ uint32_t s_lbase;
-        uint32_t total;
-        const uint32_t excl = block_excl_scan_256((uint32_t)__popc(lmask), s_lw, &total);
+        *leads = !frozen && (uint32_t)nk[u] == lo + i && event && !dead;
+        return frozen ? pend_pack(s_slot[(e - lo - (uint32_t)LT) & (uint32_t)(LT - 1)], nd[u], no[u], (uint32_t)nk[u])
+                      : FinState{(uint32_t)nk[u], no[u] | (event ? kFinEvent : 0u) | (dead ? kFinDead : 0u)};
+    };
+    __shared__ uint32_t s_lw[4];
+    __shared__ uint32_t s_lbase;
+    const uint32_t shard = blockIdx.x & (kLeaderShards - 1);
+    uint32_t lmask = 0;
+    if constexpr (DEAD) {
+#pragma unroll
+        for (int u = 0; u < PER; u++) {
+            const uint32_t i = threadIdx.x + u * 256;
+            if (i >= cnt) continue;
+            const uint32_t e = np[u];
+            const bool frozen = (e - lo) >= cnt;
+            const uint32_t li = (uint32_t)nk[u] - lo;
+            const bool dead = dead_count != nullptr && !frozen && li < cnt && (s_dead[li] & 1u) != 0;
+            const bool event = (uint32_t)(nk[u] >> 32) != kNoKey;
+            fin[lo + i] = frozen ? pend_pack(s_slot[(e - lo - (uint32_t)LT) & (uint32_t)(LT - 1)], nd[u], no[u], (uint32_t)nk[u])
+                                 : FinState{(uint32_t)nk[u], no[u] | (event ? kFinEvent : 0u) | (dead ? kFinDead : 0u)};
+            if (!frozen && (uint32_t)nk[u] == lo + i && event && !dead) lmask |= 1u << u;
+        }
+        if (leader_list) {
+            uint32_t total;
+            const uint32_t excl = block_excl_scan_256((uint32_t)__popc(lmask), s_lw, &total);
+            if (total) {
+                if (threadIdx.x == 0) s_lbase = atomicAdd(&leader_count[shard], total);
+                __syncthreads();
+                uint32_t slot = s_lbase + excl;
+                while (lmask) {
+                    const int u = __ffs(lmask) - 1;
+                    lmask &= lmask - 1;
+                    leader_list[(size_t)shard * leader_cap + slot++] = lo + threadIdx.x + (uint32_t)u * 256u;
+                }
+            }
+        }
+    } else {
+        uint32_t excl = 0, total = 0;
+        uint32_t lbase;
+        if (leader_list) {
+#pragma unroll
+            for (int u = 0; u < PER; u++) {
+                bool leads;
+                (void)final_of(u, &leads);
+                if (threadIdx.x + u * 256 < cnt && leads) lmask |= 1u << u;
+            }
+            excl = block_excl_scan_256<true>((uint32_t)__popc(lmask), s_lw, &total);
+            if (total && threadIdx.x == 0) {
+                uint32_t sh = shard;
+                asm volatile("" : "+v"(sh));
+                lbase = atomicAdd(&leader_count[sh], total);
+            }
+        }
+#pragma unroll
+        for (int u = 0; u < PER; u++) {
+            const uint32_t i = threadIdx.x + u * 256;
+            bool leads;
+            if (i < cnt) fin[lo + i] = final_of(u, &leads);
+        }
+        asm volatile("" ::: "memory");
         if (total) {
-            const uint32_t shard = blockIdx.x & (kLeaderShards - 1);
-            if (threadIdx.x == 0) s_lbase = atomicAdd(&leader_count[shard], total);
-            __syncthreads();
+            if (threadIdx.x == 0) s_lbase = lbase;
+            lds_barrier();
             uint32_t slot = s_lbase + excl;
             while (lmask) {
                 const int u = __ffs(lmask) - 1;
@@ -1514,35 +1595,39 @@
     return hipGetLastError();
 }
 
-size_t tile_mask_offset_bytes(uint32_t W, uint32_t H, uint32_t n_frames);
-size_t tile_darts_bytes(uint32_t W, uint32_t H, uint32_t n_frames) { return tile_mask_offset_bytes(W, H, n_frames) + (size_t)dart_tiles(W, H) * n_frames * kCountHalves * 8; }
-size_t tile_off_offset(uint32_t W, uint32_t H, uint32_t n_frames) { return (size_t)dart_tiles(W, H) * n_frames; }
-size_t tile_mask_offset_bytes(uint32_t W, uint32_t H, uint32_t n_frames) { return ((size_t)dart_tiles(W, H) * n_frames * 4 * (1 + kCountHalves) + 7) & ~(size_t)7; }
+size_t tile_mask_offset_bytes(uint32_t W, uint32_t H, uint32_t n_frames) { return ((size_t)dart_tiles(W, H) * n_frames * 4 * kCountHalves + 7) & ~(size_t)7; }
+size_t tile_list_offset_bytes(uint32_t W, uint32_t H, uint32_t n_frames) { return tile_mask_offset_bytes(W, H, n_frames) + (size_t)dart_tiles(W, H) * n_frames * kCountHalves * 8; }
+size_t tile_darts_bytes(uint32_t W, uint32_t H, uint32_t n_frames) { return tile_list_offset_bytes(W, H, n_frames) + (size_t)dart_tiles(W, H) * n_frames * 8 + (size_t)n_frames * 4; }
 
 hipError_t launch_dart_count(hipStream_t st, const uint64_t* bits, int W, int H, uint32_t first_frame, uint32_t n_frames,
                              unsigned long long* frame_darts, uint32_t* tile_darts, uint64_t plan_cap, uint32_t* frame_base, uint32_t* plan,
                              void* zero_p, size_t zero_bytes ) {
     const uint32_t tiles_x = dart_tiles_x((uint32_t)W), tiles_y = ((uint32_t)H + kTileRows - 1) / kTileRows;
     const uint32_t wpr = words_per_row((uint32_t)W);
-    uint32_t* h1 = tile_darts + (size_t)tiles_x * tiles_y * n_frames * 2;
+    uint32_t* h1 = tile_darts + (size_t)tiles_x * tiles_y * n_frames;
     unsigned long long* tmask = reinterpret_cast<unsigned long long*>(reinterpret_cast<uint8_t*>(tile_darts) + tile_mask_offset_bytes((uint32_t)W, (uint32_t)H, n_frames));
+    uint2* tlist = reinterpret_cast<uint2*>(reinterpret_cast<uint8_t*>(tile_darts) + tile_list_offset_bytes((uint32_t)W, (uint32_t)H, n_frames));
     if (wpr <= 30)
         hipLaunchKernelGGL(k_dart_count<32>, dim3((tiles_y + 1) / 2, n_frames, kCountHalves), dim3(64), 0, st, bits, W, H, first_frame, frame_darts, tile_darts, h1, tmask);
     else
         hipLaunchKernelGGL(k_dart_count<64>, dim3(((wpr + kCountLanes - 1) / kCountLanes) * tiles_y, n_frames, kCountHalves), dim3(64), 0, st, bits, W, H, first_frame,
                            frame_darts, tile_darts, h1, tmask);
     hipLaunchKernelGGL(k_tile_scan, dim3(n_frames + (plan ? 1u : 0u)), dim3(256), 0, st, tile_darts, h1, tiles_x * tiles_y, first_frame,
-                       tile_darts + (size_t)tiles_x * tiles_y * n_frames, n_frames, frame_darts, (unsigned long long)plan_cap, frame_base, plan,
-                       reinterpret_cast<uint4*>(zero_p), (uint32_t)(zero_bytes / 16));
+                       tlist, reinterpret_cast<uint32_t*>(tlist + (size_t)tiles_x * tiles_y * n_frames), n_frames, frame_darts,
+                       (unsigned long long)plan_cap, frame_base, plan, reinterpret_cast<uint4*>(zero_p), (uint32_t)(zero_bytes / 16));
     return hipGetLastError();
 }
 
 hipError_t launch_dart_build(hipStream_t st, const uint64_t* bits, int W, int H, uint32_t first_frame, uint32_t n_frames,
-                             const uint32_t* frame_base, const uint32_t* tile_off, uint32_t* pix_base, const uint32_t* tile_darts, uint64_t* d_rec,
-                             uint32_t* d_succ, uint32_t n_darts, const uint32_t* n_live, int dbg, const unsigned long long* tile_mask) {
+                             const uint32_t* frame_base, uint32_t* pix_base, const uint32_t* tile_tables, uint32_t frames_total, bool all_tiles,
+                             uint64_t* d_rec, uint32_t* d_succ, uint32_t n_darts, const uint32_t* n_live, int dbg) {
     const uint32_t tiles = dart_tiles((uint32_t)W, (uint32_t)H);
-    hipLaunchKernelGGL(k_dart_assign, dim3((tiles * n_frames + 7u) / 8u * 8u), dim3(256), 0, st, bits, W, H, first_frame, frame_base, tile_off,
-                       pix_base, tile_darts, d_rec, d_succ, n_live, dbg, tile_mask, tiles, n_frames);
+    const uint8_t* tt = reinterpret_cast<const uint8_t*>(tile_tables);
+    const unsigned long long* tmask = reinterpret_cast<const unsigned long long*>(tt + tile_mask_offset_bytes((uint32_t)W, (uint32_t)H, frames_total));
+    const uint2* tlist = reinterpret_cast<const uint2*>(tt + tile_list_offset_bytes((uint32_t)W, (uint32_t)H, frames_total));
+    const uint32_t wpf = all_tiles ? tiles : (tiles + 1u) / 2u;
+    hipLaunchKernelGGL(k_dart_assign, dim3((wpf * n_frames + 7u) / 8u * 8u), dim3(256), 0, st, bits, W, H, first_frame, frame_base, pix_base,
+                       d_rec, d_succ, n_live, dbg, tmask, tiles, n_frames, tlist, reinterpret_cast<const uint32_t*>(tlist + (size_t)tiles * frames_total), wpf);
     if (dbg && dbg != 5) return hipGetLastError();
     hipLaunchKernelGGL(k_dart_link, dim3(blocks_for(n_darts, 256, 4096)), dim3(256), 0, st, W, H, first_frame, pix_base, bits, d_rec, d_succ, n_darts, n_live);
     return hipGetLastError();
diff --git a/aruco3_amd/csrc/k_decode.hip b/aruco3_amd/csrc/k_decode.hip
--- a/aruco3_amd/csrc/k_decode.hip
+++ b/aruco3_amd/csrc/k_decode.hip
@@ -351,6 +351,7 @@
     uint32_t cnt;
     const uint32_t left = resize_weights(S, n, threadIdx.x, row + 2, &cnt);
     row[0] = __uint_as_float(left); row[1] = __uint_as_float(cnt);
+    for (uint32_t i = cnt; i < max_taps; i++) row[2 + i] = 0.0f;
 }
 __global__ __launch_bounds__(64, kFcWaves) void k_projection(const uint16_t* __restrict__ fin_xy, const uint32_t* __restrict__ work,
                                                    const unsigned int* __restrict__ work_count, uint32_t S, ProjRec* __restrict__ proj) {
@@ -459,7 +460,8 @@
 template <int NT, int PT>
 __global__ __launch_bounds__(NT, kDecodeWaves) void k_decode(PixelSrc src, int W, int H, uint32_t first_frame,
                                                 const uint16_t* __restrict__ fin_xy, const uint32_t* __restrict__ work,
-                                                const unsigned int* __restrict__ work_count, uint32_t max_cand, uint32_t S, uint32_t n,
+                                                const unsigned int* __restrict__ work_count, uint32_t work_cap ,
+                                                uint32_t max_cand, uint32_t S, uint32_t n,
                                                 uint32_t max_taps, const uint64_t* __restrict__ dict, uint32_t n_codes, uint32_t tau,
                                                 int filter, const ProjRec* __restrict__ proj, const float* __restrict__ wtab, DecodeOut* __restrict__ outs,
                                                 uint8_t* __restrict__ patches , uint32_t patch_cap, uint32_t* __restrict__ per_frame , int dbg) {
@@ -472,8 +474,7 @@
     uint32_t* s_cnt = reinterpret_cast<uint32_t*>(smem + o); o += (size_t)n * 4;
     uint8_t* s_bits = smem + o;
     __shared__ uint32_t s_hist[256];
-    __shared__ float s_inv[9];
-    __shared__ int s_ok, s_have;
+    __shared__ int s_have;
     __shared__ uint32_t s_otsu;
     __shared__ uint64_t s_codes[4];
     __shared__ unsigned long long s_best[NT / 64][4];
@@ -483,26 +484,33 @@
     __shared__ int s_vt[NW];
 
     const int tid = threadIdx.x;
-    const uint32_t n_work = *work_count;
-    for (uint32_t wi = blockIdx.x; wi < n_work; wi += gridDim.x) {
-        const uint32_t slot = work[wi];
+    const uint32_t wrow = max_taps + 2u, wtot = n * wrow;
+    for (uint32_t wi = blockIdx.x;; wi += gridDim.x) {
+        const uint32_t wc = min(wi, work_cap - 1u);
+        const uint32_t n_work = *work_count;
+        const uint32_t slot = work[wc];
+        float tinv[9];
+#pragma unroll
+        for (int k = 0; k < 9; k++) tinv[k] = proj[wc].inv[k];
+        const int pok = proj[wc].ok;
+        asm volatile("" ::"s"(n_work), "s"(slot), "s"(pok), "s"(tinv[0]), "s"(tinv[1]), "s"(tinv[2]), "s"(tinv[3]), "s"(tinv[4]), "s"(tinv[5]),
+                     "s"(tinv[6]), "s"(tinv[7]), "s"(tinv[8]));
+        const bool ok = pok != 0;
+        if (wi >= n_work) break;
         const uint32_t fl = slot / max_cand;
         const uint8_t* img = src.base + (size_t)(first_frame + fl) * src.frame_stride;
         __syncthreads();
-        if (tid < 9) s_inv[tid] = proj[wi].inv[tid];
-        if (tid == 9) s_ok = proj[wi].ok;
         for (int i = tid; i < 256; i += NT) s_hist[i] = 0;
         __syncthreads();
-        const bool ok = s_ok != 0;
         const uint32_t pw = ok ? S : 1u, ph = pw;
         if (ok) {
-            for (uint32_t i = tid; i < n * (max_taps + 2); i += NT) {
-                const uint32_t oi = i / (max_taps + 2), k = i - oi * (max_taps + 2);
-                const float v = wtab[i];
+            auto put = [&](uint32_t i, float v) {
+                const uint32_t oi = i / wrow, k = i - oi * wrow;
                 if (k == 0) s_left[oi] = __float_as_uint(v);
                 else if (k == 1) s_cnt[oi] = __float_as_uint(v);
-                else if (k - 2 < __float_as_uint(wtab[(size_t)oi * (max_taps + 2) + 1])) s_w[(size_t)oi * max_taps + (k - 2)] = v;
-            }
+                else s_w[(size_t)oi * max_taps + (k - 2)] = v;
+            };
+            for (uint32_t i = tid; i < wtot; i += NT) put(i, wtab[i]);
         } else if (tid < (int)n) {
             const uint32_t oi = tid;
             uint32_t cnt;
@@ -512,8 +520,8 @@
         if (ok && dbg == 1) {
             for (uint32_t i = tid; i < S * S; i += NT) { s_patch[i] = (uint8_t)(i * 7u); atomicAdd(&s_hist[(i * 7u) & 255u], 1u); }
         } else if (ok) {
-            const float t0 = s_inv[0], t1 = s_inv[1], t2 = s_inv[2], t3 = s_inv[3], t4 = s_inv[4], t5 = s_inv[5], t6 = s_inv[6],
-                        t7 = s_inv[7], t8 = s_inv[8];
+            const float t0 = tinv[0], t1 = tinv[1], t2 = tinv[2], t3 = tinv[3], t4 = tinv[4], t5 = tinv[5], t6 = tinv[6],
+                        t7 = tinv[7], t8 = tinv[8];
             constexpr int kU = kDecodeKU;
             const uint32_t bpp = (src.fmt == A3_FMT_RGB8) ? 3u : ((src.fmt == A3_FMT_RGBA8 || src.fmt == A3_FMT_BGRA8) ? 4u : 1u);
             const unsigned long long frame_bytes = (unsigned long long)(H - 1) * src.row_stride + (unsigned long long)W * bpp;
@@ -963,17 +971,17 @@
 }
 
 hipError_t launch_decode(hipStream_t st, PixelSrc src, int W, int H, uint32_t first_frame, const uint16_t* fin_xy, const uint32_t* work,
-                         const unsigned int* work_count, uint32_t max_cand, uint32_t S, uint32_t n, uint32_t max_taps, const uint64_t* dict,
+                         const unsigned int* work_count, uint32_t n_frames , uint32_t max_cand, uint32_t S, uint32_t n, uint32_t max_taps, const uint64_t* dict,
                          uint32_t n_codes, uint32_t tau, int filter, void* proj, const float* wtab, void* outs, uint8_t* patches, uint32_t patch_cap, uint32_t* per_frame, int grid_blocks, int dbg, int few) {
     ProjRec* recs = reinterpret_cast<ProjRec*>(proj);
     if (dbg > 0 || dbg == -1000) hipLaunchKernelGGL(k_projection, dim3(256), dim3(64), 0, st, fin_xy, work, work_count, S, recs);
     const int d = dbg == -1000 ? 0 : (dbg < 0 ? -dbg : dbg);
     if (few)
         hipLaunchKernelGGL((k_decode<256, 256>), dim3(grid_blocks), dim3(256), decode_lds_bytes(S, n, max_taps), st, src, W, H, first_frame, fin_xy, work, work_count,
-                           max_cand, S, n, max_taps, dict, n_codes, tau, filter, recs, wtab, reinterpret_cast<DecodeOut*>(outs), patches, patch_cap, per_frame, d);
+                           n_frames * max_cand, max_cand, S, n, max_taps, dict, n_codes, tau, filter, recs, wtab, reinterpret_cast<DecodeOut*>(outs), patches, patch_cap, per_frame, d);
     else
         hipLaunchKernelGGL((k_decode<kDecodeThreads, 64>), dim3(grid_blocks), dim3(kDecodeThreads), decode_lds_bytes(S, n, max_taps), st, src, W, H, first_frame, fin_xy, work,
-                           work_count, max_cand, S, n, max_taps, dict, n_codes, tau, filter, recs, wtab, reinterpret_cast<DecodeOut*>(outs), patches, patch_cap,
+                           work_count, n_frames * max_cand, max_cand, S, n, max_taps, dict, n_codes, tau, filter, recs, wtab, reinterpret_cast<DecodeOut*>(outs), patches, patch_cap,
                            per_frame, d);
     return hipGetLastError();
 }
```

After: 383,700, median of 2. About the same (+0.1%).
